# rti-team-imvia/RNb-NeuS-fork

Hardware: AMD Instinct MI355X
Metric: training rays/sec at 512 rays x 128 samples/ray (higher is better)
Workload: dtype f32; 1 GPU; DiLiGenT-MV-shaped synthetic rays, wmask_rnb.conf networks (8x256 SDF MLP + 2x256 albedo MLP), train_rnb step (render_rnb), 512 rays x (64+64) samples per GPU, 3 lights, geometric init, Adam; rays_per_gpu=512, global_rays=512, samples_per_ray=128, n_lights=3, no_albedo=False, parallelism=dp1, dp_loss=single process, deterministic=False, arithmetic=x2h, operand_bits=22, train_ops=rnb_loss_rnb + rnb_adam_step (one launch each)

## Files before the change

include/rnbneus.h:

```cpp
#ifndef RNBNEUS_H
#define RNBNEUS_H

#include <stddef.h>
#include <stdint.h>

#ifdef __cplusplus
extern "C" {
#endif

#define RNB_ABI_VERSION 5
#define RNB_MAX_LIN 16

enum {
  RNB_OK = 0,
  RNB_E_INVALID = -1,
  RNB_E_WORKSPACE = -2,
  RNB_E_HIP = -3,
  RNB_E_NULL = -4
};

typedef void* rnb_stream_t;

typedef struct rnb_model_desc {
  int32_t sdf_d_in;
  int32_t sdf_d_out;
  int32_t sdf_d_hidden;
  int32_t sdf_n_layers;
  int32_t sdf_skip_in;
  int32_t sdf_multires;
  float   sdf_scale;
  int32_t sdf_weight_norm;
  int32_t col_d_feature;
  int32_t col_d_in;
  int32_t col_d_out;
  int32_t col_d_hidden;
  int32_t col_n_layers;
  int32_t col_multires_view;
  int32_t col_squeeze_out;
  int32_t col_weight_norm;
  int32_t n_samples;
  int32_t n_importance;
  int32_t up_sample_steps;
  int32_t variant;
} rnb_model_desc;

enum {
  RNB_VARIANT_BF16 = 1,
  RNB_VARIANT_DETERMINISTIC = 2,
  RNB_VARIANT_GENERIC = 4,
  RNB_VARIANT_DW_LDS = 8,
  RNB_VARIANT_DW_STAGED = 16,
  RNB_VARIANT_X3 = 32,
  RNB_VARIANT_F32_MFMA = 64,
  RNB_VARIANT_BWD_TI_SHIFT = 8,
  RNB_VARIANT_BWD_NW_SHIFT = 10,
  RNB_VARIANT_FWD_TI_SHIFT = 12,
  RNB_VARIANT_FWD_NW_SHIFT = 14,
  RNB_VARIANT_REG_TILE = 1 << 16,
  RNB_VARIANT_LDS_TILE = 1 << 17,
  RNB_VARIANT_X2H = 1 << 18,
  RNB_VARIANT_NO_X2H = 1 << 19
};

typedef struct rnb_mlp_params {
  int32_t n_lin;
  int32_t pad_;
  const float* g[RNB_MAX_LIN];
  const float* v[RNB_MAX_LIN];
  const float* b[RNB_MAX_LIN];
} rnb_mlp_params;

typedef struct rnb_mlp_grads {
  int32_t n_lin;
  int32_t pad_;
  float* g[RNB_MAX_LIN];
  float* v[RNB_MAX_LIN];
  float* b[RNB_MAX_LIN];
} rnb_mlp_grads;

int rnb_abi_version(void);
const char* rnb_build_id(void);
const char* rnb_last_error_string(void);

int rnb_packed_floats(const rnb_model_desc* desc, int64_t* n_floats);
int rnb_weightnorm_fwd(const rnb_model_desc* desc, const rnb_mlp_params* sdf, const rnb_mlp_params* color,
                       float* packed, rnb_stream_t stream);
int rnb_weightnorm_bwd(const rnb_model_desc* desc, const rnb_mlp_params* sdf, const rnb_mlp_params* color,
                       const float* packed_grad, const rnb_mlp_grads* sdf_grads,
                       const rnb_mlp_grads* color_grads, rnb_stream_t stream);

int rnb_points_workspace_bytes(const rnb_model_desc* desc, int64_t n_points, int64_t* bytes);
int rnb_sdf_forward(const rnb_model_desc* desc, const float* packed, const float* pts, int64_t n,
                    float* sdf_out, float* feat_out, void* ws, size_t ws_bytes, rnb_stream_t stream);
int rnb_sdf_gradient(const rnb_model_desc* desc, const float* packed, const float* pts, int64_t n,
                     float* grad_out, float* sdf_out, void* ws, size_t ws_bytes, rnb_stream_t stream);
int rnb_color_forward(const rnb_model_desc* desc, const float* packed, const float* pts,
                      const float* normals, const float* feats, int64_t n, float* out, void* ws,
                      size_t ws_bytes, rnb_stream_t stream);

enum { RNB_POINTS_FEATURE = 1, RNB_POINTS_NORMAL = 2, RNB_POINTS_COLOR = 4 };
int rnb_points_grad_workspace_bytes(const rnb_model_desc* desc, int64_t n_points, int32_t flags, int64_t* bytes);
int rnb_sdf_forward_save(const rnb_model_desc* desc, const float* packed, const float* pts, int64_t n,
                         int32_t flags, float* sdf_out, float* feat_out, float* nrm_out, void* ws, size_t ws_bytes,
                         rnb_stream_t stream);
int rnb_sdf_backward(const rnb_model_desc* desc, const float* packed, int64_t n, int32_t flags, const float* sdf_bar,
                     const float* feat_bar, const float* nrm_bar, float* packed_grad, float* x_bar, void* ws,
                     size_t ws_bytes, rnb_stream_t stream);
int rnb_color_forward_save(const rnb_model_desc* desc, const float* packed, const float* pts, const float* normals,
                           const float* feats, int64_t n, float* out, void* ws, size_t ws_bytes, rnb_stream_t stream);
int rnb_color_backward(const rnb_model_desc* desc, const float* packed, int64_t n, const float* alb_bar,
                       float* packed_grad, float* feat_bar, float* nrm_bar, float* pts_bar, void* ws, size_t ws_bytes,
                       rnb_stream_t stream);

typedef struct rnb_grid_desc {
  float bound_min[3];
  float bound_max[3];
  int32_t resolution;
  int32_t x_begin, x_end;
  float out_scale;
} rnb_grid_desc;
int rnb_sdf_grid_workspace_bytes(const rnb_model_desc* desc, const rnb_grid_desc* grid, int64_t* bytes);
int rnb_sdf_grid(const rnb_model_desc* desc, const float* packed, const rnb_grid_desc* grid, float* volume,
                 void* ws, size_t ws_bytes, rnb_stream_t stream);

typedef struct rnb_sparse_grid_desc {
  int32_t brick;
  float threshold;
  float margin;
} rnb_sparse_grid_desc;
int rnb_sdf_grid_sparse_workspace_bytes(const rnb_model_desc* desc, const rnb_grid_desc* grid,
                                        const rnb_sparse_grid_desc* sparse, int64_t* bytes);
int rnb_sdf_grid_sparse_seed(const rnb_model_desc* desc, const float* packed, const rnb_grid_desc* grid,
                             const rnb_sparse_grid_desc* sparse, void* ws, size_t ws_bytes, int64_t* n_listed,
                             rnb_stream_t stream);
int rnb_sdf_grid_sparse_round(const rnb_model_desc* desc, const float* packed, const rnb_grid_desc* grid,
                              const rnb_sparse_grid_desc* sparse, float* volume, void* ws, size_t ws_bytes, int64_t first,
                              int64_t count, int64_t* n_listed, rnb_stream_t stream);
int rnb_sdf_grid_sparse_finish(const rnb_model_desc* desc, const rnb_grid_desc* grid, const rnb_sparse_grid_desc* sparse,
                               float* volume, void* ws, size_t ws_bytes, uint8_t* brick_mask, rnb_stream_t stream);

int rnb_up_sample_step(const float* rays_o, const float* rays_d, const float* z_in, const float* sdf_in,
                       int64_t B, int32_t n, int32_t n_new, float inv_s, float* new_z, int32_t* inds,
                       float* z_out, int32_t* sort_index, rnb_stream_t stream);
int rnb_gather_sdf(const float* sdf_old, const float* sdf_new, const int32_t* sort_index, int64_t B,
                   int32_t n, int32_t n_new, float* sdf_out, rnb_stream_t stream);
int rnb_sample_workspace_bytes(const rnb_model_desc* desc, int64_t B, int64_t* bytes);
int rnb_sample_rays(const rnb_model_desc* desc, const float* packed, const float* rays_o,
                    const float* rays_d, const float* near, const float* far, const float* t_rand,
                    int64_t B, float* z_vals_out, void* ws, size_t ws_bytes, rnb_stream_t stream);

enum {
  RNB_MODE_CORE = 0,
  RNB_MODE_MVPS = 1,
  RNB_FLAG_RELU_SHADING = 2,
  RNB_FLAG_NO_ALBEDO = 4,
  RNB_FLAG_LIGHT_PER_RAY = 8,
  RNB_FLAG_FORWARD_ONLY = 16,
  RNB_FLAG_INPUT_GRADS = 32
};

typedef struct rnb_render_args {
  int64_t B;
  int32_t S;
  int32_t n_lights;
  int32_t flags;
  float   cos_anneal_ratio;
  const float* rays_o;
  const float* rays_d;
  const float* z_vals;
  const float* lights_dir;
  const float* background_rgb;
  const float* variance;
// ... 106 lines not shown
```

rnb-neus-fork_amd/csrc/api.hip:

```cpp
#include <math.h>
#include <stdlib.h>

#include "rnb_internal.h"

using namespace rnb;

#define RNB_API extern "C" __attribute__((visibility("default")))

#define RNB_REQUIRE(p, name) \
  if (!(p)) RNB_FAIL(RNB_E_NULL, name " is NULL")

#if __has_include("../build/build_id.h")
#include "../build/build_id.h"
#endif
#ifndef RNB_BUILD_ID
#define RNB_BUILD_ID "unknown"
#endif

RNB_API int rnb_abi_version(void) { return RNB_ABI_VERSION; }
RNB_API const char* rnb_build_id(void) { return RNB_BUILD_ID; }
RNB_API const char* rnb_last_error_string(void) { return rnb::last_error(); }

RNB_API int rnb_packed_floats(const rnb_model_desc* desc, int64_t* n_floats) {
  RNB_REQUIRE(n_floats, "n_floats");
  Layout L;
  RNB_TRY(make_layout(desc, &L));
  *n_floats = L.total_all;
  return RNB_OK;
}

RNB_API int rnb_weightnorm_fwd(const rnb_model_desc* desc, const rnb_mlp_params* sdf, const rnb_mlp_params* color,
                               float* packed, rnb_stream_t stream) {
  RNB_REQUIRE(packed, "packed");
  Layout L;
  RNB_TRY(make_layout(desc, &L));
  RNB_TRY(weightnorm_fwd(desc, L, sdf, color, packed, (hipStream_t)stream));
  if (is_bf16(L)) RNB_TRY(bf16_pack_weights(L, packed, (hipStream_t)stream));
  if (is_x3(L)) RNB_TRY(x3_pack_weights(L, packed, (hipStream_t)stream));
  return RNB_OK;
}

RNB_API int rnb_weightnorm_bwd(const rnb_model_desc* desc, const rnb_mlp_params* sdf, const rnb_mlp_params* color,
                               const float* packed_grad, const rnb_mlp_grads* sdf_grads,
                               const rnb_mlp_grads* color_grads, rnb_stream_t stream) {
  RNB_REQUIRE(packed_grad, "packed_grad");
  Layout L;
  RNB_TRY(make_layout(desc, &L));
  return weightnorm_bwd(desc, L, sdf, color, packed_grad, sdf_grads, color_grads, (hipStream_t)stream);
}

static const int kPointsMode = PM_WITH_NORMAL | PM_WITH_COLOR;

RNB_API int rnb_points_workspace_bytes(const rnb_model_desc* desc, int64_t n_points, int64_t* bytes) {
  RNB_REQUIRE(bytes, "bytes");
  if (n_points < 0) RNB_FAIL(RNB_E_INVALID, "n_points < 0");
  Layout L;
  RNB_TRY(make_layout(desc, &L));
  Carver c(nullptr, 0);
  PointBufs pb;
  carve_points(L, c, n_points, kPointsMode, &pb);
  *bytes = (int64_t)c.off;
  return RNB_OK;
}

static int points_setup(const rnb_model_desc* desc, int64_t n, void* ws, size_t ws_bytes, Layout* L, PointBufs* pb) {
  RNB_TRY(make_layout(desc, L));
  RNB_REQUIRE(ws, "workspace");
  Carver c(ws, ws_bytes);
  carve_points(*L, c, n, kPointsMode, pb);
  if (!c.ok) RNB_FAIL(RNB_E_WORKSPACE, "workspace too small: need %zu bytes, have %zu", c.off, ws_bytes);
  pb->smax = nullptr;
  return RNB_OK;
}

static int forward_points(const Layout& L, const float* packed, const float* pts, int64_t n, PointBufs& pb,
                          bool save, bool need_feat, bool reverse_follows, float* feat_dense, hipStream_t s) {
  switch (L.route.sdf) {
    case SDF_BF16:
      RNB_TRY(bf16_forward(L, packed, pts, n, pb, save, need_feat, s, nullptr, save && need_feat && L.route.color == COLOR_BF16));
      break;
    case SDF_FUSED:
      RNB_TRY(fused_forward(L, packed, pts, n, pb, save, need_feat, s));
      break;
    case SDF_LAYERS:
      RNB_TRY(launch_pe_points(L, pts, n, pb, s));
      return sweep_forward(L, packed, pb, need_feat, reverse_follows, feat_dense, s);
  }
  if (need_feat && feat_dense) RNB_TRY(launch_copy_cols(pb.cin, L.Cinp, L.F, n, feat_dense, s));
  return RNB_OK;
}

static int reverse_points(const Layout& L, const float* packed, PointBufs& pb, bool store_ge, hipStream_t s) {
  switch (L.route.sdf) {
    case SDF_BF16: return bf16_reverse(L, packed, pb, s);
    case SDF_FUSED: return fused_reverse(L, packed, pb, s, store_ge);
    case SDF_LAYERS: break;
  }
  return sweep_reverse(L, packed, pb, s);
}

static int color_points(const Layout& L, const float* packed, PointBufs& pb, const float* pts, hipStream_t s) {
  switch (L.route.color) {
    case COLOR_BF16: return bf16_color_forward(L, packed, pb, pts, s);
    case COLOR_H2: return color_h2_forward(L, packed, pb, pts, pb.nrm, s);
    case COLOR_LAYERS: return sweep_color(L, packed, pb, pts, pb.nrm, 4, s);
    case COLOR_NONE: break;
  }
  RNB_FAIL(RNB_E_INVALID, "model has no albedo network");
}

RNB_API int rnb_sdf_forward(const rnb_model_desc* desc, const float* packed, const float* pts, int64_t n,
                            float* sdf_out, float* feat_out, void* ws, size_t ws_bytes, rnb_stream_t stream) {
  RNB_REQUIRE(packed, "packed");
  RNB_REQUIRE(pts, "pts");
  RNB_REQUIRE(sdf_out, "sdf_out");
  if (n <= 0) return n == 0 ? RNB_OK : (set_error("n < 0"), RNB_E_INVALID);
  hipStream_t s = (hipStream_t)stream;
  Layout L;
  PointBufs pb;
  RNB_TRY(points_setup(desc, n, ws, ws_bytes, &L, &pb));
  RNB_TRY(forward_points(L, packed, pts, n, pb, false, feat_out != nullptr, false, feat_out, s));
// ... 891 lines not shown
```

rnb-neus-fork_amd/csrc/backward.hip:

```cpp
#include "gemm.hip.h"
#include "rnb_internal.h"

namespace rnb {

__global__ __launch_bounds__(64) void nbar_geb_kernel(const float* __restrict__ x4, const float* __restrict__ nrm,
                                                      const float* __restrict__ nbar_in,
                                                      const float* __restrict__ cinb, int Cinp, int blk_off,
                                                      int pen_off, int multires_view, int with_color, int multires,
                                                      int Ep, int64_t M, int64_t Mp, float* __restrict__ geb,
                                                      unsigned* __restrict__ amax) {
  extern __shared__ float tile[];
  const int lane = threadIdx.x;
  const int64_t r0 = (int64_t)blockIdx.x * 64, row = r0 + lane;
  float nb[3] = {0.f, 0.f, 0.f};
  if (with_color) {
    const int Wc = Cinp - blk_off;
    tile_load64(cinb, Cinp, r0, blk_off, Wc, tile, lane);
    __builtin_amdgcn_wave_barrier();
    if (row < M) {
      const float* g = tile + lane * (Wc + 1) + (pen_off - blk_off);
#pragma unroll
      for (int d = 0; d < 3; ++d) nb[d] = nbar_in[row * 4 + d] + g[d];
      float f = 1.f;
      int c = 3;
      for (int k = 0; k < multires_view; ++k) {
#pragma unroll
        for (int d = 0; d < 3; ++d) {
          float s, co;
          sincosf(nrm[row * 4 + d] * f, &s, &co);
          nb[d] += f * (g[c + d] * co - g[c + 3 + d] * s);
        }
        c += 6;
        f *= 2.f;
      }
    }
    __builtin_amdgcn_wave_barrier();
  } else if (row < M) {
#pragma unroll
    for (int d = 0; d < 3; ++d) nb[d] = nbar_in[row * 4 + d];
  }
  float* o = tile + lane * (Ep + 1);
  o[0] = nb[0]; o[1] = nb[1]; o[2] = nb[2];
  float gm = fmaxf(fmaxf(fabsf(nb[0]), fabsf(nb[1])), fabsf(nb[2]));
  int c = 3;
  float f = 1.f;
  for (int k = 0; k < multires; ++k) {
#pragma unroll
    for (int d = 0; d < 3; ++d) {
      float s, co;
      sincosf(x4[row * 4 + d] * f, &s, &co);
      const float v0 = f * co * nb[d], v1 = -f * s * nb[d];
      o[c + d] = v0;
      o[c + 3 + d] = v1;
      gm = fmaxf(gm, fmaxf(fabsf(v0), fabsf(v1)));
    }
    c += 6;
    f *= 2.f;
  }
  for (; c < Ep; ++c) o[c] = 0.f;
  if (amax != nullptr) amax_commit(amax, gm, lane);
  __builtin_amdgcn_wave_barrier();
  tile_store64(geb, Ep, r0, 0, Ep, tile, lane);
}

__global__ __launch_bounds__(512) void sdf_head_bwd_kernel(const float* __restrict__ a, const float* __restrict__ ulast,
                                                           const float* __restrict__ ucol, int ntiles,
                                                           int Hp, int H, const float* __restrict__ sbar,
                                                           float inv_scale, int64_t M, int rows_per_blk,
                                                           float* __restrict__ dwsdf, float* __restrict__ dbsdf,
                                                           float* __restrict__ part_w, float* __restrict__ part_b) {
  __shared__ double red[64][33];
  __shared__ double redb[64];
  const int tid = threadIdx.x, cg = tid & 7, ph = tid >> 3;
  const int kl = cg * 4, k0 = blockIdx.y * 32 + kl;
  const int64_t r0 = (int64_t)blockIdx.x * rows_per_blk;
  const int64_t r1 = min(M, r0 + rows_per_blk);
  double s[4] = {0.0, 0.0, 0.0, 0.0}, sb = 0.0;
#pragma unroll 4
  for (int64_t row = r0 + ph; row < r1; row += 64) {
    const float t = sbar[row] * inv_scale;
    if (cg == 0) sb += (double)t;
    const vf4 av = *reinterpret_cast<const vf4*>(a + row * Hp + k0);
    if (ulast != nullptr) {
      const vf4 uv = *reinterpret_cast<const vf4*>(ulast + row * Hp + k0);
#pragma unroll
      for (int j = 0; j < 4; ++j) s[j] += (double)(t * av[j] + uv[j]);
    } else {
#pragma unroll
      for (int j = 0; j < 4; ++j) s[j] += (double)(t * av[j]);
    }
  }
  if (ulast == nullptr && blockIdx.x == 0) {
    for (int tile = ph; tile < ntiles; tile += 64) {
      const vf4 uv = *reinterpret_cast<const vf4*>(ucol + (size_t)tile * Hp + k0);
#pragma unroll
      for (int j = 0; j < 4; ++j) s[j] += (double)uv[j];
    }
  }
#pragma unroll
  for (int j = 0; j < 4; ++j) red[ph][kl + j] = s[j];
  if (cg == 0) redb[ph] = sb;
  __syncthreads();
  if (tid < 32) {
    double t = 0.0;
    for (int q = 0; q < 64; ++q) t += red[q][tid];
    const int col = blockIdx.y * 32 + tid;
    if (part_w != nullptr) part_w[(size_t)blockIdx.x * Hp + col] = col < H ? (float)t : 0.f;
    else if (col < H) atomicAdd(dwsdf + col, (float)t);
  } else if (tid == 32 && blockIdx.y == 0) {
    double t = 0.0;
    for (int q = 0; q < 64; ++q) t += redb[q];
    if (part_b != nullptr) part_b[blockIdx.x] = (float)t;
    else atomicAdd(dbsdf, (float)t);
  }
}

__global__ void sdf_xbar_kernel(const float* __restrict__ x4, const float* __restrict__ ebar, const float* __restrict__ ge,
                                const float* __restrict__ nbar, int Ep, int multires, float scale, int64_t M,
                                float* __restrict__ xbar) {
  const int64_t row = (int64_t)blockIdx.x * blockDim.x + threadIdx.x;
  if (row >= M) return;
  const float* eb = ebar + row * Ep;
  float acc[3] = {eb[0], eb[1], eb[2]};
  float f = 1.f;
  int c = 3;
  for (int k = 0; k < multires; ++k) {
#pragma unroll
    for (int d = 0; d < 3; ++d) {
      float sn, co;
      sincosf(x4[row * 4 + d] * f, &sn, &co);
      acc[d] += f * (eb[c + d] * co - eb[c + 3 + d] * sn);
      if (ge != nullptr) {
        const float* g = ge + row * Ep;
        acc[d] -= f * f * (g[c + d] * sn + g[c + 3 + d] * co) * nbar[row * 4 + d];
      }
    }
    c += 6;
    f *= 2.f;
  }
#pragma unroll
  for (int d = 0; d < 3; ++d) xbar[row * 3 + d] = scale * acc[d];
}

__global__ void color_input_bwd_kernel(const float* __restrict__ cinb, int Cinp, int F, int pev, int multires_view,
                                       const float* __restrict__ p4, const float* __restrict__ n4, int64_t M,
                                       float* __restrict__ pbar, float* __restrict__ nbar) {
  const int64_t row = (int64_t)blockIdx.x * blockDim.x + threadIdx.x;
  if (row >= M) return;
  for (int which = 0; which < 2; ++which) {
    float* out = which ? nbar : pbar;
    if (out == nullptr) continue;
    const float* g = cinb + row * Cinp + F + which * pev;
    const float* v = (which ? n4 : p4) + row * 4;
    float t[3] = {g[0], g[1], g[2]};
    float f = 1.f;
    int c = 3;
    for (int k = 0; k < multires_view; ++k) {
#pragma unroll
      for (int d = 0; d < 3; ++d) {
        float sn, co;
        sincosf(v[d] * f, &sn, &co);
// ... 111 lines not shown
```

rnb-neus-fork_amd/csrc/composite.hip:

```cpp
#include "rnb_internal.h"

namespace rnb {

constexpr int kMaxL = kMaxRenderLights;

__device__ inline float sigm(float x) { return 1.0f / (1.0f + expf(-x)); }

__device__ inline float inv_s_from_variance(const float* variance, bool* inside_clip) {
  const float raw = expf(variance[0] * 10.0f);
  if (inside_clip) *inside_clip = (raw >= 1e-6f) && (raw <= 1e6f);
  return clamp_nan(raw, 1e-6f, 1e6f);
}

__global__ void fine_points_kernel(const float* __restrict__ rays_o, const float* __restrict__ rays_d,
                                   const float* __restrict__ z, int64_t B, int S, float sample_dist,
                                   float* __restrict__ pts, float* __restrict__ dists, unsigned* __restrict__ smax) {
  int64_t i = (int64_t)blockIdx.x * blockDim.x + threadIdx.x;
  if (smax != nullptr && i < SMAX_SLOTS) smax[i] = 0u;
  if (i >= B * S) return;
  const int64_t b = i / S;
  const int j = (int)(i - b * S);
  const float zz = z[i];
  const float dd = j + 1 < S ? z[i + 1] - zz : sample_dist;
  const float mid = zz + dd * 0.5f;
// ... 35 lines not shown
  st.e_prev = s - ic * delta * 0.5f;
  st.pc = sigm(st.e_prev * inv_s);
  st.nc = sigm(st.e_next * inv_s);
  st.raw = (st.pc - st.nc + 1e-5f) / (st.pc + 1e-5f);
  st.alpha = clamp_nan(st.raw, 0.f, 1.f);
  return st;
}

__device__ inline void load_light(const CompArgs& a, int l, int64_t b, float (&Lv)[3]) {
  const float* p = (a.flags & RNB_FLAG_LIGHT_PER_RAY) ? a.lights + ((int64_t)l * a.B + b) * 3 : a.lights + l * 3;
  Lv[0] = p[0]; Lv[1] = p[1]; Lv[2] = p[2];
}

__global__ __launch_bounds__(64) void composite_fwd_kernel(CompArgs a) {
  const int lane = threadIdx.x;
  const int64_t b = blockIdx.x;
  const int S = a.S;
  const bool mvps = (a.flags & RNB_MODE_MVPS) != 0;
  const bool relu_sh = (a.flags & RNB_FLAG_RELU_SHADING) != 0;
  const bool no_alb = (a.flags & RNB_FLAG_NO_ALBEDO) != 0;
  const float inv_s = inv_s_from_variance(a.variance, nullptr);
  const float d0 = a.rays_d[b * 3], d1 = a.rays_d[b * 3 + 1], d2 = a.rays_d[b * 3 + 2];
  float Lv[kMaxL][3];
  if (mvps)
    for (int l = 0; l < a.L; ++l) load_light(a, l, b, Lv[l]);

  float carry = 1.0f;
  float col[kMaxL][4];
#pragma unroll
  for (int l = 0; l < kMaxL; ++l)
#pragma unroll
    for (int c = 0; c < 4; ++c) col[l][c] = 0.f;
  float wsum = 0.f, wmax = -1.f, gnum = 0.f, gden = 0.f;

  for (int j0 = 0; j0 < S; j0 += 64) {
    const int j = j0 + lane;
    const bool on = j < S;
    const int64_t p = b * S + (on ? j : S - 1);
    const float s = a.sdf[p];
    const float n0 = a.nrm[p * 4], n1 = a.nrm[p * 4 + 1], n2 = a.nrm[p * 4 + 2];
    const SampleState st = eval_sample(s, n0, n1, n2, d0, d1, d2, a.dists[p], inv_s, a.cos_anneal);
    const float x = on ? (1.0f - st.alpha + 1e-7f) : 1.0f;
    const float incl = wave_scan_mul(x, lane);
    float excl = __shfl_up(incl, 1, 64);
    if (lane == 0) excl = 1.0f;
    const float T = carry * excl;
    carry = carry * __shfl(incl, 63, 64);
    const float w = on ? st.alpha * T : 0.f;
    const float px = a.pts[p * 3], py = a.pts[p * 3 + 1], pz = a.pts[p * 3 + 2];
    const float pn = sqrtf(px * px + py * py + pz * pz);
    const float nn = sqrtf(n0 * n0 + n1 * n1 + n2 * n2);
    if (on) {
      a.weights[p] = w;
      a.cdf[p] = st.pc;
      a.gradients[p * 3] = n0; a.gradients[p * 3 + 1] = n1; a.gradients[p * 3 + 2] = n2;
      a.inside[p] = pn < 1.0f ? 1.f : 0.f;
      if (a.sdf_out) a.sdf_out[p] = s;
      if (a.albedo_out)
        for (int c = 0; c < a.C; ++c) a.albedo_out[p * a.C + c] = a.alb[p * 4 + c];
      wsum += w;
      wmax = max_nan(wmax, w);
      {
        const float relax = pn < 1.2f ? 1.f : 0.f;
        gnum += relax * ((nn - 1.0f) * (nn - 1.0f));
        gden += relax;
      }
      float al[4];
#pragma unroll
      for (int c = 0; c < 4; ++c) al[c] = no_alb ? 1.0f : a.alb[p * 4 + c];
      if (mvps) {
        for (int l = 0; l < a.L; ++l) {
          float sh = n0 * Lv[l][0] + n1 * Lv[l][1] + n2 * Lv[l][2];
          if (relu_sh) sh = relu_nan(sh);
          const float ws = w * sh;
#pragma unroll
          for (int c = 0; c < 4; ++c) col[l][c] = fmaf(al[c], ws, col[l][c]);
        }
      } else {
#pragma unroll
        for (int c = 0; c < 4; ++c) col[0][c] = fmaf(a.alb[p * 4 + c], w, col[0][c]);
      }
    }
  }
  wsum = wave_sum(wsum);
  wmax = wave_max(wmax);
  gnum = wave_sum(gnum);
  gden = wave_sum(gden);
  const int nl = mvps ? a.L : 1;
  for (int l = 0; l < nl; ++l)
    for (int c = 0; c < a.C; ++c) {
      float v = wave_sum(col[l][c]);
      if (lane == 0) {
        if (mvps) a.color_fine[((int64_t)l * a.B + b) * a.C + c] = v;
        else if (c < 3) {
          if (a.bg) v += a.bg[c] * (1.0f - wsum);
          a.color_fine[b * 3 + c] = v;
        }
      }
    }
  if (lane == 0) {
    a.weight_sum[b] = wsum;
    a.weight_max[b] = wmax;
    a.s_val[b] = 1.0f / inv_s;
    a.gerr_part[b * 2] = gnum;
    a.gerr_part[b * 2 + 1] = gden;
  }
}

__global__ __launch_bounds__(64) void composite_maps_kernel(CompMapsArgs g) {
  const CompArgs& a = g.f;
  const int lane = threadIdx.x;
  const int64_t b = blockIdx.x;
  const int S = a.S;
  const bool mvps = (a.flags & RNB_MODE_MVPS) != 0;
  const bool relu_sh = (a.flags & RNB_FLAG_RELU_SHADING) != 0;
  const bool no_alb = (a.flags & RNB_FLAG_NO_ALBEDO) != 0;
  const bool want_color = a.color_fine != nullptr;
  const float inv_s = inv_s_from_variance(a.variance, nullptr);
  const float d0 = a.rays_d[b * 3], d1 = a.rays_d[b * 3 + 1], d2 = a.rays_d[b * 3 + 2];
  float Lv[kMaxL][3];
  if (mvps && want_color)
    for (int l = 0; l < a.L; ++l) load_light(a, l, b, Lv[l]);

  float carry = 1.0f;
  float col[kMaxL][4];
#pragma unroll
  for (int l = 0; l < kMaxL; ++l)
#pragma unroll
    for (int c = 0; c < 4; ++c) col[l][c] = 0.f;
  float wsum = 0.f, wmax = -1.f;
  float nacc[3] = {0.f, 0.f, 0.f}, aacc[4] = {0.f, 0.f, 0.f, 0.f}, dacc = 0.f;

  for (int j0 = 0; j0 < S; j0 += 64) {
    const int j = j0 + lane;
    const bool on = j < S;
    const int64_t p = b * S + (on ? j : S - 1);
    const float s = a.sdf[p];
    const float n0 = a.nrm[p * 4], n1 = a.nrm[p * 4 + 1], n2 = a.nrm[p * 4 + 2];
    const SampleState st = eval_sample(s, n0, n1, n2, d0, d1, d2, a.dists[p], inv_s, a.cos_anneal);
    const float x = on ? (1.0f - st.alpha + 1e-7f) : 1.0f;
    const float incl = wave_scan_mul(x, lane);
    float excl = __shfl_up(incl, 1, 64);
    if (lane == 0) excl = 1.0f;
    const float T = carry * excl;
    carry = carry * __shfl(incl, 63, 64);
    const float w = on ? st.alpha * T : 0.f;
    const float px = a.pts[p * 3], py = a.pts[p * 3 + 1], pz = a.pts[p * 3 + 2];
    const float pn = sqrtf(px * px + py * py + pz * pz);
    if (on) {
      wsum += w;
      wmax = max_nan(wmax, w);
      if (g.normal) {
        const float wi = w * (pn < 1.0f ? 1.f : 0.f);
        nacc[0] = fmaf(wi, n0, nacc[0]); nacc[1] = fmaf(wi, n1, nacc[1]); nacc[2] = fmaf(wi, n2, nacc[2]);
      }
      if (g.albedo) {
#pragma unroll
        for (int c = 0; c < 4; ++c) aacc[c] = fmaf(a.alb[p * 4 + c], w, aacc[c]);
      }
      if (g.depth) dacc = fmaf(w, g.z[p] + a.dists[p] * 0.5f, dacc);
      if (want_color) {
        float al[4];
#pragma unroll
        for (int c = 0; c < 4; ++c) al[c] = no_alb ? 1.0f : a.alb[p * 4 + c];
        if (mvps) {
          for (int l = 0; l < a.L; ++l) {
            float sh = n0 * Lv[l][0] + n1 * Lv[l][1] + n2 * Lv[l][2];
            if (relu_sh) sh = relu_nan(sh);
            const float ws = w * sh;
#pragma unroll
            for (int c = 0; c < 4; ++c) col[l][c] = fmaf(al[c], ws, col[l][c]);
          }
        } else {
#pragma unroll
          for (int c = 0; c < 4; ++c) col[0][c] = fmaf(a.alb[p * 4 + c], w, col[0][c]);
        }
      }
    }
  }
  wsum = wave_sum(wsum);
  wmax = wave_max(wmax);
  if (want_color) {
    const int nl = mvps ? a.L : 1;
    for (int l = 0; l < nl; ++l)
      for (int c = 0; c < a.C; ++c) {
        float v = wave_sum(col[l][c]);
        if (lane == 0) {
          if (mvps) a.color_fine[((int64_t)l * a.B + b) * a.C + c] = v;
          else if (c < 3) {
            if (a.bg) v += a.bg[c] * (1.0f - wsum);
            a.color_fine[b * 3 + c] = v;
          }
        }
      }
  }
  if (g.normal) {
#pragma unroll
    for (int d = 0; d < 3; ++d) {
      const float v = wave_sum(nacc[d]);
      if (lane == 0) g.normal[b * 3 + d] = v;
    }
  }
  if (g.albedo) {
    for (int c = 0; c < a.C; ++c) {
      const float v = wave_sum(aacc[c]);
      if (lane == 0) g.albedo[b * a.C + c] = v;
    }
  }
  if (g.depth) {
    const float v = wave_sum(dacc);
    if (lane == 0) g.depth[b] = v;
  }
  if (lane == 0) {
    if (a.weight_sum) a.weight_sum[b] = wsum;
    if (a.weight_max) a.weight_max[b] = wmax;
  }
}

__global__ __launch_bounds__(256) void gerr_finalize_kernel(const float* __restrict__ part, int64_t B,
                                                            float* __restrict__ gerr, float* __restrict__ den_out,
                                                            float* __restrict__ partial) {
  __shared__ float rn[4], rd[4];
  float n = 0.f, d = 0.f;
  for (int64_t i = threadIdx.x; i < B; i += 256) { n += part[i * 2]; d += part[i * 2 + 1]; }
  n = wave_sum(n);
  d = wave_sum(d);
  if ((threadIdx.x & 63) == 0) { rn[threadIdx.x >> 6] = n; rd[threadIdx.x >> 6] = d; }
  __syncthreads();
  if (threadIdx.x == 0) {
    const float nn = rn[0] + rn[1] + rn[2] + rn[3];
    const float ds = rd[0] + rd[1] + rd[2] + rd[3];
    const float dd = ds + 1e-5f;
    gerr[0] = nn / dd;
    den_out[0] = dd;
    if (partial) { partial[0] = nn; partial[1] = ds; }
  }
}


template <bool IG>
__device__ __forceinline__ void composite_bwd_body(const CompBwdArgs& g) {
  __shared__ float sAlpha[kMaxS], sT[kMaxS], sWbar[kMaxS], sSuf[kMaxS];
  if (g.amax_to_zero != nullptr && blockIdx.x == 0) {
    static_assert(AMAX_SLOTS <= 64, "one wave zeroes the slots");
    if ((int)threadIdx.x < AMAX_SLOTS) g.amax_to_zero[threadIdx.x] = 0u;
  }
  const CompArgs& a = g.f;
  const int lane = threadIdx.x;
  const int64_t b = blockIdx.x;
  const int S = a.S;
  const bool mvps = (a.flags & RNB_MODE_MVPS) != 0;
  const bool relu_sh = (a.flags & RNB_FLAG_RELU_SHADING) != 0;
  const bool no_alb = (a.flags & RNB_FLAG_NO_ALBEDO) != 0;
  const float inv_s = inv_s_from_variance(a.variance, nullptr);
  const float c_an = a.cos_anneal;
  const float d0 = a.rays_d[b * 3], d1 = a.rays_d[b * 3 + 1], d2 = a.rays_d[b * 3 + 2];
  float Lv[kMaxL][3], Cb[kMaxL][4];
#pragma unroll
  for (int l = 0; l < kMaxL; ++l)
#pragma unroll
    for (int c = 0; c < 4; ++c) Cb[l][c] = 0.f;
  const int nl = mvps ? a.L : 1;
  if (mvps)
    for (int l = 0; l < a.L; ++l) load_light(a, l, b, Lv[l]);
  if (g.g_color) {
    for (int l = 0; l < nl; ++l)
      for (int c = 0; c < (mvps ? a.C : 3); ++c)
        Cb[l][c] = mvps ? g.g_color[((int64_t)l * a.B + b) * a.C + c] : g.g_color[b * 3 + c];
  }
  const float g_wsum = g.g_weight_sum ? g.g_weight_sum[b] : 0.f;
  const float g_wmax = g.g_weight_max ? g.g_weight_max[b] : 0.f;
  float bg_dot = 0.f;
  if (!mvps && a.bg) bg_dot = Cb[0][0] * a.bg[0] + Cb[0][1] * a.bg[1] + Cb[0][2] * a.bg[2];

  float carry = 1.0f;
  float wmax = -1.f;
  int wmax_j = 0;
  float lbar[kMaxL][3];
  float wsum_ig = 0.f;
  if constexpr (IG) {
#pragma unroll
    for (int l = 0; l < kMaxL; ++l) lbar[l][0] = lbar[l][1] = lbar[l][2] = 0.f;
  }
  for (int j0 = 0; j0 < S; j0 += 64) {
    const int j = j0 + lane;
    const bool on = j < S;
    const int64_t p = b * S + (on ? j : S - 1);
    const float n0 = a.nrm[p * 4], n1 = a.nrm[p * 4 + 1], n2 = a.nrm[p * 4 + 2];
    const SampleState st = eval_sample(a.sdf[p], n0, n1, n2, d0, d1, d2, a.dists[p], inv_s, c_an);
    const float x = on ? (1.0f - st.alpha + 1e-7f) : 1.0f;
    const float incl = wave_scan_mul(x, lane);
    float excl = __shfl_up(incl, 1, 64);
    if (lane == 0) excl = 1.0f;
    const float T = carry * excl;
    carry = carry * __shfl(incl, 63, 64);
    if (on) {
      const float w = st.alpha * T;
      float wb = g_wsum + (g.g_weights ? g.g_weights[p] : 0.f);
      float nb0 = 0.f, nb1 = 0.f, nb2 = 0.f;
      float ab[4] = {0.f, 0.f, 0.f, 0.f};
      float al[4];
#pragma unroll
      for (int c = 0; c < 4; ++c) al[c] = (mvps && no_alb) ? 1.0f : a.alb[p * 4 + c];
      if (mvps) {
        for (int l = 0; l < a.L; ++l) {
          const float sh_raw = n0 * Lv[l][0] + n1 * Lv[l][1] + n2 * Lv[l][2];
          const float sh = relu_sh ? fmaxf(sh_raw, 0.f) : sh_raw;
          float ca = 0.f;
#pragma unroll
          for (int c = 0; c < 4; ++c) {
            ca = fmaf(Cb[l][c], al[c], ca);
            ab[c] = fmaf(Cb[l][c], w * sh, ab[c]);
          }
          wb = fmaf(ca, sh, wb);
          float shb = ca * w;
          if (relu_sh && !(sh_raw > 0.f)) shb = 0.f;
          nb0 = fmaf(shb, Lv[l][0], nb0); nb1 = fmaf(shb, Lv[l][1], nb1); nb2 = fmaf(shb, Lv[l][2], nb2);
          if constexpr (IG) if (g.ig_light) { lbar[l][0] = fmaf(shb, n0, lbar[l][0]); lbar[l][1] = fmaf(shb, n1, lbar[l][1]); lbar[l][2] = fmaf(shb, n2, lbar[l][2]); }
        }
        if (no_alb) { ab[0] = ab[1] = ab[2] = ab[3] = 0.f; }
      } else {
#pragma unroll
        for (int c = 0; c < 3; ++c) { wb = fmaf(Cb[0][c], al[c], wb); ab[c] = Cb[0][c] * w; }
        wb -= bg_dot;
      }
      sAlpha[j] = st.alpha;
      sT[j] = T;
      sWbar[j] = wb;
      g.nbar[p * 4] = nb0; g.nbar[p * 4 + 1] = nb1; g.nbar[p * 4 + 2] = nb2; g.nbar[p * 4 + 3] = 0.f;
#pragma unroll
      for (int c = 0; c < 4; ++c) g.albbar[p * 4 + c] = ab[c];
      if (w > wmax) { wmax = w; wmax_j = j; }
      if constexpr (IG) wsum_ig += w;
    }
  }
  if constexpr (IG) {
    if (g.ig_light) {
      for (int l = 0; l < a.L; ++l)
#pragma unroll
        for (int d = 0; d < 3; ++d) {
          const float v = wave_sum(lbar[l][d]);
          if (lane == 0) g.ig_light[((int64_t)l * a.B + b) * 3 + d] = v;
        }
    }
    if (g.ig_bg) {
      const float ws = wave_sum(wsum_ig);
      if (lane == 0)
        for (int c = 0; c < 3; ++c) g.ig_bg[b * 3 + c] = Cb[0][c] * (1.0f - ws);
    }
  }
  if (g.g_weight_max) {
    const float m = wave_max(wmax);
    int cand = (wmax == m) ? wmax_j : 0x7fffffff;
#pragma unroll
    for (int o = 32; o > 0; o >>= 1) cand = min(cand, __shfl_xor(cand, o, 64));
    __syncthreads();
    if (lane == 0 && cand < S) sWbar[cand] += g_wmax;
  }
  __syncthreads();
  if (lane == 0) {
    double run = 0.0;
    for (int j = S - 1; j >= 0; --j) {
      sSuf[j] = (float)run;
      run += (double)sWbar[j] * (double)(sAlpha[j] * sT[j]);
    }
  }
  __syncthreads();
  const float gerr_coef = g.g_gerr ? g.g_gerr[0] / (g.gerr_den_global ? g.gerr_den_global[0] : g.gerr_den[0]) : 0.f;
  float invs_bar = 0.f;
  float cosd0 = 0.f, cosd1 = 0.f, cosd2 = 0.f;
  for (int j0 = 0; j0 < S; j0 += 64) {
    const int j = j0 + lane;
    if (j >= S) continue;
    const int64_t p = b * S + j;
    const float n0 = a.nrm[p * 4], n1 = a.nrm[p * 4 + 1], n2 = a.nrm[p * 4 + 2];
    const float delta = a.dists[p];
    const SampleState st = eval_sample(a.sdf[p], n0, n1, n2, d0, d1, d2, delta, inv_s, c_an);
    float alphabar = sWbar[j] * sT[j] - sSuf[j] / (1.0f - st.alpha + 1e-7f);
    const float rawbar = (st.raw >= 0.f && st.raw <= 1.f) ? alphabar : 0.f;
    const float den = st.pc + 1e-5f;
    float pcbar = rawbar * (1.0f / den - (st.pc - st.nc + 1e-5f) / (den * den));
    const float ncbar = -rawbar / den;
    if (g.g_cdf) pcbar += g.g_cdf[p];
    float epb = pcbar * st.pc * (1.0f - st.pc);
    float enb = ncbar * st.nc * (1.0f - st.nc);
    invs_bar += epb * st.e_prev + enb * st.e_next;
    epb *= inv_s;
    enb *= inv_s;
    g.sbar[p] = epb + enb;
    const float icbar = (enb - epb) * delta * 0.5f;
    const float tcbar = icbar * (((-st.tc * 0.5f + 0.5f) > 0.f ? 0.5f * (1.0f - c_an) : 0.f) +
                                 ((-st.tc) > 0.f ? c_an : 0.f));
    if constexpr (IG) if (g.ig_cos_d) { cosd0 = fmaf(tcbar, n0, cosd0); cosd1 = fmaf(tcbar, n1, cosd1); cosd2 = fmaf(tcbar, n2, cosd2); }
    if constexpr (IG) if (g.ig_dists) {
      const float ic = -(relu_nan(-st.tc * 0.5f + 0.5f) * (1.0f - c_an) + relu_nan(-st.tc) * c_an);
      g.ig_dists[p] = (enb - epb) * ic * 0.5f;
    }
    float nb0 = g.nbar[p * 4] + tcbar * d0, nb1 = g.nbar[p * 4 + 1] + tcbar * d1, nb2 = g.nbar[p * 4 + 2] + tcbar * d2;
    if (g.g_gerr) {
      const float px = a.pts[p * 3], py = a.pts[p * 3 + 1], pz = a.pts[p * 3 + 2];
      if (sqrtf(px * px + py * py + pz * pz) < 1.2f) {
        const float nn = sqrtf(n0 * n0 + n1 * n1 + n2 * n2);
        if (nn > 0.f) {
          const float k = gerr_coef * 2.0f * (nn - 1.0f) / nn;
          nb0 = fmaf(k, n0, nb0); nb1 = fmaf(k, n1, nb1); nb2 = fmaf(k, n2, nb2);
        }
      }
    }
    if (g.g_gradients) {
      nb0 += g.g_gradients[p * 3]; nb1 += g.g_gradients[p * 3 + 1]; nb2 += g.g_gradients[p * 3 + 2];
    }
    g.nbar[p * 4] = nb0; g.nbar[p * 4 + 1] = nb1; g.nbar[p * 4 + 2] = nb2;
  }
  invs_bar = wave_sum(invs_bar);
  if (lane == 0) {
    if (g.g_s_val) invs_bar -= g.g_s_val[b] / (inv_s * inv_s);
    g.invs_part[b] = invs_bar;
  }
  if constexpr (IG) if (g.ig_cos_d) {
    cosd0 = wave_sum(cosd0);
    cosd1 = wave_sum(cosd1);
    cosd2 = wave_sum(cosd2);
    if (lane == 0) { g.ig_cos_d[b * 3] = cosd0; g.ig_cos_d[b * 3 + 1] = cosd1; g.ig_cos_d[b * 3 + 2] = cosd2; }
  }
}

__global__ __launch_bounds__(64) void composite_bwd_kernel(CompBwdArgs g) { composite_bwd_body<false>(g); }
__global__ __launch_bounds__(64) void composite_bwd_ig_kernel(CompBwdArgs g) { composite_bwd_body<true>(g); }

__global__ __launch_bounds__(64) void ray_input_adjoint_kernel(RayAdjArgs r) {
  const int lane = threadIdx.x;
  const int64_t b = blockIdx.x;
  const int S = r.S;
  const float d0 = r.rays_d[b * 3], d1 = r.rays_d[b * 3 + 1], d2 = r.rays_d[b * 3 + 2];
  float ob[3] = {0.f, 0.f, 0.f}, db[3] = {0.f, 0.f, 0.f};
  float carry_D = 0.f;
  for (int j0 = 0; j0 < S; j0 += 64) {
    const int j = j0 + lane;
    const bool on = j < S;
    const int64_t p = b * S + (on ? j : S - 1);
    float nt[3], pb[3];
#pragma unroll
    for (int d = 0; d < 3; ++d) nt[d] = r.nbar[p * 4 + d];
    if (r.cinb != nullptr) {
      const float* gn = r.cinb + p * r.Cinp + r.F + r.pev;
      const float* gp = r.cinb + p * r.Cinp + r.F;
#pragma unroll
// ... 151 lines not shown
```

rnb-neus-fork_amd/csrc/dw.hip.h:

```cpp
#pragma once
#include "gemm.hip.h"

namespace rnb {

struct DwPair {
  const float* X;
  int ldx;
  const float* Y;
  int ldy;
  int adj = 0;
  const unsigned* amax = nullptr;
  const unsigned* smax = nullptr;
};

template <bool GUARD, int KT>
__device__ inline void dw_main_loop(const DwPair& p, int m_begin, int m_end, int N, int K, int n_blk, int k_blk,
                                    int wm, int wn, unsigned mask, bool do_bias, double& bsum,
                                    float* __restrict__ Xs, float* __restrict__ Ys, v16f (&acc)[2][KT / 64]) {
  const int tid = threadIdx.x, lane = tid & 63;
  vf4 rx[4], ry[KT / 32];
  load_kmajor<128, GUARD>(p.X, p.ldx, m_begin, n_blk, m_end, N, tid, rx);
  load_kmajor<KT, GUARD>(p.Y, p.ldy, m_begin, k_blk, m_end, K, tid, ry);
  for (int m0 = m_begin; m0 < m_end; m0 += BK) {
    store_kmajor<128>(Xs, tid, rx);
// ... 180 lines not shown
    for (int c = 0; c < nch; c += 3) {
      RNB_DW_LOAD(2, c + 2)
      __builtin_amdgcn_sched_barrier(0);
      RNB_DW_MMA(0)
      __builtin_amdgcn_sched_barrier(0);
      RNB_DW_LOAD(0, c + 3)
      __builtin_amdgcn_sched_barrier(0);
      if (c + 1 < nch) RNB_DW_MMA(1)
      __builtin_amdgcn_sched_barrier(0);
      RNB_DW_LOAD(1, c + 4)
      __builtin_amdgcn_sched_barrier(0);
      if (c + 2 < nch) RNB_DW_MMA(2)
      __builtin_amdgcn_sched_barrier(0);
    }
#undef RNB_DW_LOAD
#undef RNB_DW_MMA
  }
  float* __restrict__ dW = J.dW;
  const int lddw = J.lddw;
  float* __restrict__ pdst = J.part ? J.part + (size_t)split * N * lddw : nullptr;
#pragma unroll
  for (int tj = 0; tj < TN; ++tj) {
    const int col = k_w + tj * 32 + i;
#pragma unroll
    for (int ti = 0; ti < 2; ++ti) {
#pragma unroll
      for (int r = 0; r < 16; ++r) {
        const int row = n_w + 2 * ((r & 3) + 8 * (r >> 2) + 4 * h) + ti;
        if (pdst) pdst[(size_t)row * lddw + col] = acc[ti][tj][r];
        else atomicAdd(dW + (size_t)row * lddw + col, acc[ti][tj][r]);
      }
    }
  }
  if (bias_wave) {
    bs0 += __shfl_xor(bs0, 32, 64);
    bs1 += __shfl_xor(bs1, 32, 64);
    if (h == 0) {
      if (J.partb) {
        J.partb[(size_t)split * N + n_w + 2 * i] = (float)bs0;
        J.partb[(size_t)split * N + n_w + 2 * i + 1] = (float)bs1;
      } else {
        atomicAdd(J.db + n_w + 2 * i, (float)bs0);
        atomicAdd(J.db + n_w + 2 * i + 1, (float)bs1);
      }
    }
  }
}

template <int DUMMY>
__global__ __launch_bounds__(256) void dw_reduce_kernel(const DwGroup g) {
  const DwJob& J = g.job[blockIdx.y];
  const size_t n = (size_t)J.N * J.K;
  const bool dense = J.K == J.lddw;
  if (J.splits > 64) {
    __shared__ double red[16][17];
    const size_t ntot = n + ((J.db != nullptr && J.partb != nullptr) ? (size_t)J.N : 0);
    const int e = threadIdx.x & 15, ph = threadIdx.x >> 4;
    for (size_t base = (size_t)blockIdx.x * 16; base < ntot; base += (size_t)gridDim.x * 16) {
      const size_t idx = base + e;
      double s[4] = {0.0, 0.0, 0.0, 0.0};
      if (idx < ntot) {
        const float* src = idx < n ? J.part + idx : J.partb + (idx - n);
        const size_t stride = idx < n ? n : (size_t)J.N;
        int sp = ph;
        for (; sp + 48 < J.splits; sp += 64) {
#pragma unroll
          for (int u = 0; u < 4; ++u) s[u] += (double)src[(size_t)(sp + 16 * u) * stride];
        }
        for (int u = 0; sp < J.splits; sp += 16, ++u) s[u] += (double)src[(size_t)sp * stride];
      }
      red[ph][e] = (s[0] + s[1]) + (s[2] + s[3]);
      __syncthreads();
      if (threadIdx.x < 16 && base + threadIdx.x < ntot) {
        const size_t i2 = base + threadIdx.x;
        double t = 0.0;
        for (int q = 0; q < 16; ++q) t += red[q][threadIdx.x];
        if (i2 < n) J.dW[dense ? i2 : (i2 / (size_t)J.K) * (size_t)J.lddw + i2 % (size_t)J.K] = (float)t;
        else J.db[i2 - n] = (float)t;
      }
      __syncthreads();
    }
    return;
  }
  for (size_t idx = (size_t)blockIdx.x * 256 + threadIdx.x; idx < n; idx += (size_t)gridDim.x * 256) {
    double s[4] = {0.0, 0.0, 0.0, 0.0};
    int sp = 0;
    for (; sp + 4 <= J.splits; sp += 4) {
#pragma unroll
      for (int u = 0; u < 4; ++u) s[u] += (double)J.part[(size_t)(sp + u) * n + idx];
    }
    for (int u = 0; sp < J.splits; ++sp, ++u) s[u] += (double)J.part[(size_t)sp * n + idx];
    const size_t dst = dense ? idx : (idx / (size_t)J.K) * (size_t)J.lddw + idx % (size_t)J.K;
    J.dW[dst] = (float)((s[0] + s[1]) + (s[2] + s[3]));
  }
  if (J.db != nullptr && J.partb != nullptr) {
    for (int r = blockIdx.x * 256 + threadIdx.x; r < J.N; r += gridDim.x * 256) {
      double s = 0.0;
      for (int sp = 0; sp < J.splits; ++sp) s += (double)J.partb[(size_t)sp * J.N + r];
      J.db[r] = (float)s;
    }
  }
}

constexpr int kStChunk = 32;
constexpr int kStOpBytes = kStChunk * 256 * 4;
constexpr int kStBufs = 2;

__device__ inline void dw_staged_issue(const DwPair& p, int m_begin, int nchunks, int chunk, char* buf, int wave, int lane) {
  const int c = chunk < nchunks ? chunk : nchunks - 1;
#pragma unroll
  for (int q = 0; q < kStChunk / 16; ++q) {
    const int u = (q * 16 + wave) * 64 + lane;
    const int row = m_begin + c * kStChunk + (u >> 6);
    const float* xs = p.X + (size_t)row * p.ldx + (u & 63) * 4;
    const float* ys = p.Y + (size_t)row * p.ldy + (u & 63) * 4;
    __builtin_amdgcn_global_load_lds((const __attribute__((address_space(1))) void*)xs,
                                     (__attribute__((address_space(3))) void*)(buf + (q * 16 + wave) * 1024), 16, 0, 0);
    __builtin_amdgcn_global_load_lds((const __attribute__((address_space(1))) void*)ys,
                                     (__attribute__((address_space(3))) void*)(buf + kStOpBytes + (q * 16 + wave) * 1024), 16, 0, 0);
  }
}

template <int DUMMY>
__global__ __launch_bounds__(1024, 1) void gemm_dw_staged_kernel(const DwGroup g) {
  __shared__ __attribute__((aligned(16))) char lds[kStBufs * 2 * kStOpBytes];
  const int tid = threadIdx.x, lane = tid & 63;
  const int wave = wave_id();
  const int wm = wave >> 2, wn = wave & 3;
  int ji = 0, begin = 0;
  for (int q = 0; q + 1 < g.njobs; ++q)
    if ((int)blockIdx.x >= g.job[q].block_end) { ji = q + 1; begin = g.job[q].block_end; }
  const DwJob& J = g.job[ji];
  const int split = (int)blockIdx.x - begin;
  if (split >= J.splits) return;
  const int m_begin = split * J.rows_per_split;
  const int m_end = min(g.M, m_begin + J.rows_per_split);
  if (m_begin >= m_end) return;
  const int nchunks = (m_end - m_begin) / kStChunk;
  const int i = lane & 31, h = lane >> 5;
  v16f acc[2][2];
  zero_acc<2>(acc);
  double bs0 = 0.0, bs1 = 0.0;
  const bool bias_wave = J.db != nullptr && wn == 0;
  for (int pi = 0; pi < J.npairs; ++pi) {
    const DwPair p = pi == 0 ? J.p1 : J.p2;
    const bool do_bias = bias_wave && pi == J.bias_pair;
    __builtin_amdgcn_s_barrier();
    dw_staged_issue(p, m_begin, nchunks, 0, lds, wave, lane);
    for (int c = 0; c < nchunks; ++c) {
      asm volatile("s_waitcnt vmcnt(0)" ::: "memory");
      __builtin_amdgcn_s_barrier();
      dw_staged_issue(p, m_begin, nchunks, c + 1, lds + ((c + 1) & 1) * 2 * kStOpBytes, wave, lane);
      const char* bx = lds + (c & 1) * 2 * kStOpBytes;
      const char* by = bx + kStOpBytes;
      float t0 = 0.f, t1 = 0.f;
      const char* ax = bx + h * 1024 + (wm * 64 + 2 * i) * 4;
      const char* ay = by + h * 1024 + (wn * 64 + i) * 4;
      vf2 a0 = *reinterpret_cast<const vf2*>(ax);
      float b00 = *reinterpret_cast<const float*>(ay), b01 = *reinterpret_cast<const float*>(ay + 128);
#pragma unroll
      for (int q = 0; q < kStChunk / 2; q += 2) {
        const vf2 a1 = *reinterpret_cast<const vf2*>(ax + (q + 1) * 2048);
        const float b10 = *reinterpret_cast<const float*>(ay + (q + 1) * 2048);
        const float b11 = *reinterpret_cast<const float*>(ay + (q + 1) * 2048 + 128);
        __builtin_amdgcn_sched_barrier(0);
        acc[0][0] = __builtin_amdgcn_mfma_f32_32x32x2f32(a0.x, b00, acc[0][0], 0, 0, 0);
        acc[1][0] = __builtin_amdgcn_mfma_f32_32x32x2f32(a0.y, b00, acc[1][0], 0, 0, 0);
        acc[0][1] = __builtin_amdgcn_mfma_f32_32x32x2f32(a0.x, b01, acc[0][1], 0, 0, 0);
        acc[1][1] = __builtin_amdgcn_mfma_f32_32x32x2f32(a0.y, b01, acc[1][1], 0, 0, 0);
        if (do_bias) { t0 += a0.x; t1 += a0.y; }
        __builtin_amdgcn_sched_barrier(0);
        if (q + 2 < kStChunk / 2) {
          a0 = *reinterpret_cast<const vf2*>(ax + (q + 2) * 2048);
          b00 = *reinterpret_cast<const float*>(ay + (q + 2) * 2048);
          b01 = *reinterpret_cast<const float*>(ay + (q + 2) * 2048 + 128);
        }
        __builtin_amdgcn_sched_barrier(0);
        acc[0][0] = __builtin_amdgcn_mfma_f32_32x32x2f32(a1.x, b10, acc[0][0], 0, 0, 0);
        acc[1][0] = __builtin_amdgcn_mfma_f32_32x32x2f32(a1.y, b10, acc[1][0], 0, 0, 0);
        acc[0][1] = __builtin_amdgcn_mfma_f32_32x32x2f32(a1.x, b11, acc[0][1], 0, 0, 0);
        acc[1][1] = __builtin_amdgcn_mfma_f32_32x32x2f32(a1.y, b11, acc[1][1], 0, 0, 0);
// ... 288 lines not shown
```

rnb-neus-fork_amd/csrc/fused.hip:

```cpp
#include <type_traits>

#include "fused_common.hip.h"

#ifndef RNB_X3_SCALAR_EPI
#define RNB_X3_SCALAR_EPI 0
#endif
#ifndef RNB_H2_SCALAR_EPI
#define RNB_H2_SCALAR_EPI 1
#endif
#ifndef RNB_H2_GUARD_AB
#define RNB_H2_GUARD_AB 0
#endif

namespace rnb {


template <int TI, bool SAVE, int NW = 4, bool X3 = false, bool H2 = false>
__global__ __launch_bounds__(64 * NW, NW == 8 ? 1 : 2) void fused_forward_kernel(FusedFwdArgs g) {
  static_assert(!H2 || X3, "x2h is a form of the split-operand path");
  constexpr float SA = H2 ? kH2ActScale : 1.f;
  constexpr int WP = H2 ? 2 : 3;
  constexpr int FT = 32 * TI;
  constexpr int NT = 64 * NW;
  constexpr int TJ = 8 / NW;
// ... 144 lines not shown
              D = vf2{0.f, 0.f};
              if constexpr (H2) am = fmaxf(am, fmaxf(fabsf(a.x), fabsf(a.y)));
            }
          }
          Y[row * FP + col] = a.x * SA;
          Y[(row + 1) * FP + col] = a.y * SA;
          if constexpr (H2 && RNB_H2_GUARD_AB != 1) h2_track2(amb, a.x, a.y);
          if (SAVE) {
            bstore(ra, voff, rowc * FH * 4, a.x);
            bstore(ra, voff, (rowc + 1) * FH * 4, a.y);
            bstore(rD, voff, rowc * FH * 4, D.x);
            bstore(rD, voff, (rowc + 1) * FH * 4, D.y);
          }
        }
      }
    };
#pragma unroll
    for (int tj = 0; tj < TJ; ++tj) {
      if (n0 + tj * 32 + 32 <= n_real) column_tile(std::true_type{}, tj);
      else column_tile(std::false_type{}, tj);
    }
    if constexpr (H2 && RNB_H2_GUARD_AB != 1) {
      am = fmaxf(am, __builtin_bit_cast(float, amb));
      h2_raise_flag(am, &ovf[l & 1], lane);
    }
    lds_barrier();
    if constexpr (H2) {
      sa = SA;
      isa = 1.f / SA;
      am_prev = am;
    }
    if constexpr (NBUF == 2) { float* t = X; X = Y; Y = t; }
  }
  if constexpr (H2 && RNB_H2_GUARD_AB == 0) {
    if (h2_flag_up(&ovf[(g.net.nh - 1) & 1])) rescale_input(am_prev, g.net.nh - 1);
  }

  {
    const float* ws = g.packed + g.net.wsdf_off;
    float w[4];
#pragma unroll
    for (int u = 0; u < 4; ++u) w[u] = ws[lane + 64 * u];
    const float bs = g.packed[g.net.bsdf_off];
    for (int rr = 0; rr < FT / NW; ++rr) {
      const int row = wave * (FT / NW) + rr;
      float s = 0.f;
#pragma unroll
      for (int u = 0; u < 4; ++u) s = fmaf(X[row * FP + lane + 64 * u], w[u], s);
#pragma unroll
      for (int o = 32; o > 0; o >>= 1) s += __shfl_xor(s, o, 64);
      if (lane == 0) {
        const float v = (H2 ? __builtin_fmaf(s, isa, bs) : s + bs) / g.net.scale;
        sweep_store_sdf(g.grid, g.sdf, row0, row, g.M, v);
      }
    }
  }
  if (g.with_feat) {
    [[maybe_unused]] const float inv = H2 ? isa * h2_iws_at(iwsv, g.net.nh) : 1.f;
    if constexpr (X3) mm.run(X, g.w3 + WP * g.net.wf_off, FH, n0, lane, acc, nullptr, 0, 0);
    else layer_mma_nt<TI, NoHook, TJ>(X, g.packed + g.net.wf_off, FH, n0, lane, acc);
    const float* bias = g.packed + g.net.bf_off;
    const BufRsrc rc = tile_rsrc(g.cin + (size_t)row0 * g.net.Cinp, FT * g.net.Cinp * 4);
    const unsigned rowb = (unsigned)g.net.Cinp * 4u;
#pragma unroll
    for (int tj = 0; tj < TJ; ++tj) {
      const int col = n0 + tj * 32 + cl;
      if (col < g.net.F) {
        const float bc = bias[col];
        const unsigned voff = (unsigned)(4 * h) * rowb + (unsigned)col * 4u;
#pragma unroll
        for (int ti = 0; ti < TI; ++ti) {
#pragma unroll
          for (int r = 0; r < 16; ++r) {
            const int rowc = ti * 32 + (r & 3) + 8 * (r >> 2);
            bstore(rc, voff, rowc * rowb, H2 ? __builtin_fmaf(acc[ti][tj][r], inv, bc) : acc[ti][tj][r] + bc);
          }
        }
      }
    }
  }
}

constexpr int kMaxX3 = 4 * RNB_MAX_LIN + 2;
struct X3Entry { long long off; int N, K, unit_begin, tperm, id, tr; };
struct X3Table { int n, total_units; X3Entry e[kMaxX3]; };
__global__ __launch_bounds__(256) void x3_pack_kernel(const float* __restrict__ src, X3Table t, x3raw* __restrict__ dst,
                                                      H2Tab* __restrict__ tab) {
  __shared__ float wmx[4];
  const int u = blockIdx.x * 256 + threadIdx.x;
  const bool live = u < t.total_units;
  int ei = 0;
  while (ei + 1 < t.n && u >= t.e[ei + 1].unit_begin) ++ei;
  const X3Entry en = t.e[ei];
  float m = 0.f;
  if (live) {
    const int lu = u - en.unit_begin;
    const int frag = lu >> 6, lane = lu & 63;
    const int nks = en.K >> 4;
    const int nt = frag / nks, ks = frag - nt * nks;
    const int c = lane & 31, h = lane >> 5;
    const float* sp = src + en.off + (size_t)(nt * 32 + c) * en.K + ks * 16 + h * (en.tperm ? 4 : 8);
    const vf4 x0 = *reinterpret_cast<const vf4*>(sp), x1 = *reinterpret_cast<const vf4*>(sp + (en.tperm ? 8 : 4));
    vu4x hi, mid, lo;
    x3_split8(x0, x1, hi, mid, lo);
    x3raw* dp = dst + 3 * en.off + ((size_t)frag * 3 * 64 + lane) * 8;
    *reinterpret_cast<vu4x*>(dp) = hi;
    *reinterpret_cast<vu4x*>(dp + 512) = mid;
    *reinterpret_cast<vu4x*>(dp + 1024) = lo;
    m = fmaxf(fmaxf(fmaxf(fabsf(x0.x), fabsf(x0.y)), fmaxf(fabsf(x0.z), fabsf(x0.w))),
              fmaxf(fmaxf(fabsf(x1.x), fabsf(x1.y)), fmaxf(fabsf(x1.z), fabsf(x1.w))));
  }
  if (tab == nullptr) return;
  const bool rec = live && en.id >= 0 && !en.tr;
  const int blk0 = blockIdx.x * 256;
  const bool whole = en.unit_begin <= blk0 && blk0 + 256 <= en.unit_begin + en.N * en.K / 8;
#pragma unroll
  for (int o = 32; o > 0; o >>= 1) m = fmaxf(m, __shfl_xor(m, o, 64));
  if (!whole) {
    if (rec && (threadIdx.x & 63) == 0) amax_tile_commit(tab->wmax + en.id, m);
    return;
  }
  if ((threadIdx.x & 63) == 0) wmx[threadIdx.x >> 6] = m;
  __syncthreads();
  if (rec && threadIdx.x == 0) amax_tile_commit(tab->wmax + en.id, fmaxf(fmaxf(wmx[0], wmx[1]), fmaxf(wmx[2], wmx[3])));
}
__device__ inline float x2h_weight_scale(unsigned mbits, float& inv) {
  float s = kH2WScale;
  inv = 1.f / kH2WScale;
  const int ef = (int)(mbits >> 23);
  if (ef >= 127 + 6 && ef < 255) x2h_dyn_scale(mbits, s, inv);
  return s;
}
__global__ void x2h_pack_kernel(const float* __restrict__ src, X3Table t, x3raw* __restrict__ dst, H2Tab* __restrict__ tab) {
  const int u = blockIdx.x * blockDim.x + threadIdx.x;
  if (u >= t.total_units) return;
  int ei = 0;
  while (ei + 1 < t.n && u >= t.e[ei + 1].unit_begin) ++ei;
  const X3Entry en = t.e[ei];
  const int lu = u - en.unit_begin;
  const int frag = lu >> 6, lane = lu & 63;
  const int nks = en.K >> 4;
  const int nt = frag / nks, ks = frag - nt * nks;
  const int c = lane & 31, h = lane >> 5;
  float inv;
  const float sw = x2h_weight_scale(tab->wmax[en.id], inv);
  if (lu == 0 && !en.tr) { tab->ws[en.id] = sw; tab->iws[en.id] = inv; }
  const float* sp = src + en.off + (size_t)(nt * 32 + c) * en.K + ks * 16 + h * (en.tperm ? 4 : 8);
  vu4x hi, lo;
  x2h_split8(*reinterpret_cast<const vf4*>(sp) * sw, *reinterpret_cast<const vf4*>(sp + (en.tperm ? 8 : 4)) * sw, hi, lo);
  x3raw* dp = dst + 2 * en.off + ((size_t)frag * 2 * 64 + lane) * 8;
  *reinterpret_cast<vu4x*>(dp) = hi;
  *reinterpret_cast<vu4x*>(dp + 512) = lo;
}
int x3_pack_weights(const Layout& L, float* packed, hipStream_t s) {
  x3raw* dst = reinterpret_cast<x3raw*>(packed + L.total);
  X3Table t;
  t.n = 0;
  t.total_units = 0;
  auto add = [&](long long off, int N, int K, int tperm, int id, int tr) {
    if (off < 0 || N <= 0 || K <= 0) return;
    X3Entry& e = t.e[t.n++];
    e.off = off; e.N = N; e.K = K; e.unit_begin = t.total_units; e.tperm = tperm; e.id = id; e.tr = tr;
    t.total_units += N * K / 8;
  };
  for (int l = 0; l < L.nh; ++l) {
    add(L.hid[l].w_off, L.hid[l].Np, L.hid[l].Kp, 1, l, 0);
    add(L.hid[l].wT_off, L.hid[l].Kp, L.hid[l].Np, 1, l, 1);
  }
  if (L.F > 0) {
    add(L.feat.w_off, L.feat.Np, L.feat.Kp, 1, L.nh, 0);
    add(L.feat.wT_off, L.feat.Kp, L.feat.Np, 1, L.nh, 1);
  }
  for (int l = 0; l < L.nc; ++l) {
    add(L.col[l].w_off, L.col[l].Np, L.col[l].Kp, 0, L.nh + 1 + l, 0);
    add(L.col[l].wT_off, L.col[l].Kp, L.col[l].Np, 0, L.nh + 1 + l, 1);
  }
  H2Tab* tab = is_x2h(L) ? h2_tab(L, packed) : nullptr;
  hipLaunchKernelGGL(x3_pack_kernel, dim3((unsigned)((t.total_units + 255) / 256)), dim3(256), 0, s, packed, t, dst, tab);
  RNB_CHECK_LAUNCH();
  if (is_x2h(L)) {
    for (int q = 0; q < t.n; ++q) t.e[q].tperm = 1;
    hipLaunchKernelGGL(x2h_pack_kernel, dim3((unsigned)((t.total_units + 255) / 256)), dim3(256), 0, s, packed, t,
                       x2h_mirror(L, packed), tab);
    RNB_CHECK_LAUNCH();
  }
  return RNB_OK;
}

bool fused_supported(const Layout& L) {
  if (L.Hp != FH || L.H != FH) return false;
  if (L.Ep > 64 || L.pe > FEP) return false;
  if (L.nh < 1) return false;
  for (int l = 0; l < L.nh; ++l)
    if (L.hid[l].Np != FH || (L.hid[l].Kp != FH && l != 0)) return false;
  if (L.F > FH || (L.F > 0 && L.Fp != FH)) return false;
  return true;
}

int fused_forward(const Layout& L, const float* packed, const float* pts, int64_t M, PointBufs& pb, bool save,
                  bool need_feat, hipStream_t s, const GridGen* grid) {
  const int64_t fam_rows = family_rows_of(grid, pb.Mp);
  if (!save && use_reg_tile(L, fam_rows)) return sweep_mv_forward(L, packed, pts, M, pb, save, need_feat, s, grid);
  const bool h2 = is_x2h(L);
  FusedFwdArgs g;
  memset(&g, 0, sizeof(g));
  g.net = sdf_net_args(L);
  if (grid) g.grid = *grid;
  g.pts = pts;
  g.M = M;
  g.packed = packed;
  g.w3 = h2 ? x2h_mirror(L, packed) : reinterpret_cast<const x3raw*>(packed + L.total);
  for (int l = 0; l < L.nh; ++l) {
    g.a[l] = pb.a[l];
    g.D[l] = pb.D[l];
  }
  g.with_feat = need_feat ? 1 : 0;
  g.cin = pb.cin;
  g.sdf = pb.sdf;
  g.x4 = pb.x;
  g.e = pb.e;
  g.h2tab = h2 ? h2_tab(L, packed) : nullptr;
  g.smax = (save && h2) ? pb.smax : nullptr;
  ProfScope prof(sdf_sweep_flops(L, M, 0, true, need_feat), s, save ? "F_sweep(save)" : "F_sweep(forward_only)");
  const int force_ti = L.knob(RNB_VARIANT_FWD_TI_SHIFT);
  const bool small = force_ti ? (force_ti == 1) : (fam_rows / 64 < 512);
  const int force_nw = L.knob(RNB_VARIANT_FWD_NW_SHIFT);
  const bool wide = force_nw ? (force_nw == 2) : (fam_rows / 32 <= 256);
  pick_c<1, 0>(save, [&](auto save_c) {
    pick_c<2, 1, 0>(h2 ? 2 : is_x3(L) ? 1 : 0, [&](auto ar_c) {
      auto launch = [&](auto ti_c, auto nw_c) {
        constexpr int TI = decltype(ti_c)::value, NW = decltype(nw_c)::value, AR = decltype(ar_c)::value;
        hipLaunchKernelGGL((fused_forward_kernel<TI, decltype(save_c)::value != 0, NW, AR >= 1, AR == 2>),
                           dim3((unsigned)(pb.Mp / (32 * TI))), dim3(64 * NW), 0, s, g);
      };
      if (!small) launch(std::integral_constant<int, 2>{}, std::integral_constant<int, 4>{});
      else pick_c<8, 4>(wide ? 8 : 4, [&](auto nw_c) { launch(std::integral_constant<int, 1>{}, nw_c); });
    });
  });
  RNB_CHECK_LAUNCH();
  return RNB_OK;
}

}
```

rnb-neus-fork_amd/csrc/fused_bwd.hip:

```cpp
#include "fused_common.hip.h"

namespace rnb {


struct FusedBwdArgs {
  const float* packed;
  const x3raw* w3;
  SdfNetArgs net;
  float* D[RNB_MAX_LIN];
  float* gz[RNB_MAX_LIN];
  float* u[RNB_MAX_LIN + 1];
  long long M;
  float* ucol;
  float* zR[RNB_MAX_LIN];
  float* zb[RNB_MAX_LIN];
  const float* x4;
  float* nrm;
  const float* geb;
  const float* sbar;
  const float* fbar;
  int ld_fbar;
  unsigned* amax;
  const H2Tab* h2tab;
  unsigned* smax;
// ... 432 lines not shown
  for (int l = g.net.nh - 1; l >= 0; --l) {
    const int lane_e = opaque_lane(lane);
    const int h = lane_e >> 5;
    const int n_real = g.net.n_real[l];
    const bool head = (l == g.net.nh - 1);
    const int par = l & 1;
    const BufRsrc rzb = tile_rsrc(g.zb[l] + (size_t)row0 * FH, BT * FH * 4);
    if (head) {
      for_each_acc<TI, TJ>(n0, lane_e, [&](int tj, int ti, int r, int col, int rowc, int row) {
        acc[ti][tj][r] = fmaf(g.sbar[row0 + row] * g.net.inv_scale, g.packed[g.net.wsdf_off + col], acc[ti][tj][r] * unscale);
      });
      unscale = 1.f;
    }
    for_each_acc_split<TI, TJ>(
        n0, lane_e, n_real,
        [&](int tj, int ti, int r, int col, int rowc, int row) {
          const float zb = fmaf(acc[ti][tj][r] * unscale, aD.v[ti][tj][r], aZ.v[ti][tj][r]);
          bstore(rzb, (unsigned)(4 * h * FH + col) * 4u, rowc * FH * 4, zb);
          acc[ti][tj][r] = zb;
        },
        [&](int tj, int ti, int r, int col, int rowc, int row) {
          const float zb = col < n_real ? fmaf(acc[ti][tj][r] * unscale, aD.v[ti][tj][r], aZ.v[ti][tj][r]) : 0.f;
          bstore(rzb, (unsigned)(4 * h * FH + col) * 4u, rowc * FH * 4, zb);
          acc[ti][tj][r] = zb;
        });
    {
      const float mr = wave_max(acc_absmax<TI, TJ>(acc, lane_e, rows_ok));
      if (lane_e == 0) wm[par][wave] = mr;
    }
    lds_barrier();
    float s, inv;
    const float tmax = tile_scale<NW>(wm[par], s, inv);
    if (tid == 0 && g.amax != nullptr) amax_tile_commit(g.amax + AMAX_ZB + l, tmax);
    if (l == 0) break;
    for_each_acc<TI, TJ>(n0, lane_e, [&](int tj, int ti, int r, int col, int rowc, int row) {
      X[row * FP + col] = acc[ti][tj][r] * s;
    });
    lds_barrier();
    if constexpr (LATE) {
      mm.request(g.w3 + 2 * g.net.wT_off[l], FH, n0, lane);
      mm.run(X, g.w3 + 2 * g.net.wT_off[l], FH, n0, lane, acc, nullptr, 0, 0);
      prefetch_tile<TI, TJ>(g.D[l - 1], row0, n0, opaque_lane(lane), aD);
      prefetch_tile<TI, TJ>(g.zR[l - 1], row0, n0, opaque_lane(lane), aZ);
    } else {
      mm.run(X, g.w3 + 2 * g.net.wT_off[l], FH, n0, lane, acc, l > 1 ? g.w3 + 2 * g.net.wT_off[l - 1] : nullptr, FH, n0, [&]() {
        prefetch_tile<TI, TJ>(g.D[l - 1], row0, n0, lane, aD);
        prefetch_tile<TI, TJ>(g.zR[l - 1], row0, n0, lane, aZ);
      });
    }
    unscale = inv * h2_iws_at(iwsv, l);
  }
}

static void fill_args(const Layout& L, const float* packed, PointBufs& pb, FusedBwdArgs& g) {
  memset(&g, 0, sizeof(g));
  g.net = sdf_net_args(L);
  g.packed = packed;
  g.w3 = reinterpret_cast<const x3raw*>(packed + L.total);
  for (int l = 0; l < L.nh; ++l) {
    g.D[l] = pb.D[l];
    g.gz[l] = pb.gz[l];
    g.zR[l] = pb.zR[l];
    g.zb[l] = pb.zb[l];
  }
  for (int l = 1; l <= L.nh; ++l) g.u[l] = pb.u[l];
  g.M = pb.M;
  g.x4 = pb.x;
  g.nrm = pb.nrm;
  g.geb = pb.geb;
  g.sbar = pb.sbar;
  g.amax = is_x2h(L) ? pb.amax : nullptr;
  g.h2tab = is_x2h(L) ? h2_tab(L, packed) : nullptr;
}

template <class F>
static void pick_tile(const Layout& L, const PointBufs& pb, F&& f) {
  const int kt = L.knob(RNB_VARIANT_BWD_TI_SHIFT), kw = L.knob(RNB_VARIANT_BWD_NW_SHIFT);
  const int ti = kt == 1 || kt == 2 ? kt : (is_x3(L) ? 2 : 1), nw = kw == 1 ? 4 : kw == 2 ? 8 : (is_x3(L) ? 4 : 8);
  pick_c<2, 1>(ti, [&](auto ti_c) {
    pick_c<8, 4>(nw, [&](auto nw_c) { f(ti_c, nw_c, dim3((unsigned)(pb.Mp / (32 * ti_c))), dim3(64 * nw_c)); });
  });
}

int fused_reverse(const Layout& L, const float* packed, PointBufs& pb, hipStream_t s, bool store_ge) {
  FusedBwdArgs g;
  fill_args(L, packed, pb, g);
  g.ge_out = store_ge ? pb.ge : nullptr;
  if (is_x2h(L)) {
    g.w3 = x2h_mirror(L, packed);
    g.smax = pb.smax;
  }
  ProfScope prof(sdf_sweep_flops(L, pb.M, 0, false, false), s, "R_sweep");
  pick_tile(L, pb, [&](auto ti_c, auto nw_c, dim3 grid, dim3 block) {
    pick_c<2, 1, 0>(is_x2h(L) ? 2 : is_x3(L) ? 1 : 0, [&](auto ar_c) {
      constexpr int AR = decltype(ar_c)::value;
      hipLaunchKernelGGL((fused_reverse_kernel<decltype(ti_c)::value, decltype(nw_c)::value, AR >= 1, AR == 2>), grid, block, 0, s, g);
    });
  });
  RNB_CHECK_LAUNCH();
  return RNB_OK;
}

int fused_ra(const Layout& L, const float* packed, PointBufs& pb, hipStream_t s, int* u_tiles) {
  FusedBwdArgs g;
  fill_args(L, packed, pb, g);
  ProfScope prof(sdf_sweep_flops(L, pb.M, 0, false, false), s, "RA_sweep");
  pick_tile(L, pb, [&](auto ti_c, auto nw_c, dim3 grid, dim3 block) {
    if (u_tiles != nullptr) {
      g.ucol = pb.u[L.nh];
      *u_tiles = (int)grid.x;
    }
    pick_c<1, 0>(is_x3(L), [&](auto x3_c) {
      hipLaunchKernelGGL((fused_ra_kernel<decltype(ti_c)::value, decltype(nw_c)::value, decltype(x3_c)::value != 0>), grid, block, 0, s, g);
    });
  });
  RNB_CHECK_LAUNCH();
  return RNB_OK;
}

int fused_fb(const Layout& L, const float* packed, PointBufs& pb, bool with_color, hipStream_t s) {
  FusedBwdArgs g;
  fill_args(L, packed, pb, g);
  g.fbar = with_color ? pb.cinb : nullptr;
  g.ld_fbar = L.Cinp;
  ProfScope prof(sdf_sweep_flops(L, pb.M, 1, false, with_color), s, "FB_sweep");
  pick_tile(L, pb, [&](auto ti_c, auto nw_c, dim3 grid, dim3 block) {
    constexpr int TI = decltype(ti_c)::value, NW = decltype(nw_c)::value;
    if constexpr (TI == 2) {
      if (is_x2h(L)) {
        g.w3 = x2h_mirror(L, packed);
        hipLaunchKernelGGL((fused_fb_h2_kernel<NW>), grid, block, 0, s, g);
        return;
      }
    }
    pick_c<1, 0>(is_x3(L), [&](auto x3_c) {
      hipLaunchKernelGGL((fused_fb_kernel<TI, NW, decltype(x3_c)::value != 0>), grid, block, 0, s, g);
    });
  });
  RNB_CHECK_LAUNCH();
  return RNB_OK;
}

}
```

rnb-neus-fork_amd/csrc/layers.hip:

```cpp
#include "gemm.hip.h"
#include "rnb_internal.h"

namespace rnb {


__global__ void pe_points_kernel(const float* __restrict__ pts, int64_t M, int64_t Mp, float scale, int multires,
                                 int Ep, float* __restrict__ x4, float* __restrict__ e) {
  int64_t row = (int64_t)blockIdx.x * blockDim.x + threadIdx.x;
  if (row >= Mp) return;
  float x[3] = {0.f, 0.f, 0.f};
  if (row < M) {
    x[0] = pts[row * 3 + 0] * scale;
    x[1] = pts[row * 3 + 1] * scale;
    x[2] = pts[row * 3 + 2] * scale;
  }
  x4[row * 4 + 0] = x[0]; x4[row * 4 + 1] = x[1]; x4[row * 4 + 2] = x[2]; x4[row * 4 + 3] = 0.f;
  float* er = e + row * Ep;
  er[0] = x[0]; er[1] = x[1]; er[2] = x[2];
  int c = 3;
  float f = 1.f;
  for (int k = 0; k < multires; ++k) {
#pragma unroll
    for (int d = 0; d < 3; ++d) {
      float s, co;
// ... 361 lines not shown
#pragma unroll
      for (int c = 0; c < 4; ++c) v[c] = fmaf(sb, w[c], v[c]);
    }
    vf4 zb;
#pragma unroll
    for (int c = 0; c < 4; ++c) zb[c] = col + c < n_real ? fmaf(v[c], Dv[c], zr[c]) : 0.f;
    st4(zb_prev + o, zb);
  }
};
struct EpiReluMask {
  const float* ac_prev;
  float* out;
  int ld;
  int n_real;
  __device__ void apply4(int row, int col, vf4 v) const {
    const size_t o = (size_t)row * ld + col;
    const vf4 a = ld4(ac_prev + o);
    vf4 r;
#pragma unroll
    for (int c = 0; c < 4; ++c) r[c] = (col + c < n_real && a[c] > 0.f) ? v[c] : 0.f;
    st4(out + o, r);
  }
};
struct EpiStore {
  float* out;
  int ld;
  __device__ void apply4(int row, int col, vf4 v) const { st4(out + (size_t)row * ld + col, v); }
};

struct EpiSkipPE {
  float* ebar;
  int Ep, k_split, pe;
  __device__ void apply4(int row, int col, vf4 v) const {
#pragma unroll
    for (int c = 0; c < 4; ++c) {
      const int cc = col + c;
      if (cc >= k_split && cc < k_split + pe) ebar[(size_t)row * Ep + (cc - k_split)] = v[c];
    }
  }
};


template <bool B_KMAJOR, class Epi>
static int launch_rows(const float* A, int lda, const float* W, int ldw, int64_t Mp, int N, int K, const Epi& epi,
                       double flops, hipStream_t s, bool x3 = false, const x3raw* W3 = nullptr, unsigned* amax = nullptr,
                       int64_t m_real = 0, const char* tag = "layer_gemm") {
  ProfScope prof(flops, s, tag);
  if constexpr (!B_KMAJOR) {
    if (x3 && W3 != nullptr && N % 32 == 0 && N <= 512 && K % 32 == 0 && Mp % 128 == 0) {
      if (N <= 256) hipLaunchKernelGGL((gemm_rows_x3m_kernel<1, Epi>), dim3((unsigned)(Mp / 128)), dim3(512), 0, s, A, lda, W3, N, K, epi, amax, (long long)m_real);
      else hipLaunchKernelGGL((gemm_rows_x3m_kernel<2, Epi>), dim3((unsigned)(Mp / 128)), dim3(512), 0, s, A, lda, W3, N, K, epi, amax, (long long)m_real);
      RNB_CHECK_LAUNCH();
      return RNB_OK;
    }
    if (amax != nullptr) RNB_FAIL(RNB_E_INVALID, "layer GEMM %d x %d: the x2h maxima were requested from a kernel that does not record them", N, K);
    if (x3 && N >= 256 && K % XK == 0) {
      dim3 grid((unsigned)(Mp / BM), (unsigned)((N + 255) / 256));
      if (N % 256 == 0) hipLaunchKernelGGL((gemm_rows_x3_kernel<256, false, Epi>), grid, dim3(256), 0, s, A, lda, W, ldw, N, K, epi);
      else hipLaunchKernelGGL((gemm_rows_x3_kernel<256, true, Epi>), grid, dim3(256), 0, s, A, lda, W, ldw, N, K, epi);
      RNB_CHECK_LAUNCH();
      return RNB_OK;
    }
  }
  if (N >= 256) {
    dim3 grid((unsigned)(Mp / BM), (unsigned)((N + 255) / 256));
    if (N % 256 == 0)
      hipLaunchKernelGGL((gemm_rows_kernel<B_KMAJOR, 256, false, Epi>), grid, dim3(256), 0, s, A, lda, W, ldw, N, K, epi);
    else
      hipLaunchKernelGGL((gemm_rows_kernel<B_KMAJOR, 256, true, Epi>), grid, dim3(256), 0, s, A, lda, W, ldw, N, K, epi);
  } else {
    dim3 grid((unsigned)(Mp / BM), (unsigned)((N + 127) / 128));
    if (N % 128 == 0)
      hipLaunchKernelGGL((gemm_rows_kernel<B_KMAJOR, 128, false, Epi>), grid, dim3(256), 0, s, A, lda, W, ldw, N, K, epi);
    else
      hipLaunchKernelGGL((gemm_rows_kernel<B_KMAJOR, 128, true, Epi>), grid, dim3(256), 0, s, A, lda, W, ldw, N, K, epi);
  }
  RNB_CHECK_LAUNCH();
  return RNB_OK;
}

static inline const x3raw* x3_mirror(const Layout& L, const float* packed, int64_t off) {
  if (!is_x3(L) || off < 0) return nullptr;
  return reinterpret_cast<const x3raw*>(packed + L.total) + 3 * off;
}

int launch_pe_points(const Layout& L, const float* pts, int64_t M, PointBufs& pb, hipStream_t s) {
  hipLaunchKernelGGL(pe_points_kernel, dim3(blocks_for(pb.Mp, 256)), dim3(256), 0, s, pts, M, pb.Mp, L.sdf_scale,
                     L.multires, L.Ep, pb.x, pb.e);
  RNB_CHECK_LAUNCH();
  return RNB_OK;
}

int sweep_forward(const Layout& L, const float* packed, PointBufs& pb, bool need_feat, bool need_gz_last,
                  float* feat_dense, hipStream_t s) {
  for (int l = 0; l < L.nh; ++l) {
    const Lin& ln = L.hid[l];
    const float* in = l == 0 ? pb.e : pb.a[l - 1];
    const int lda = l == 0 ? L.Ep : L.Hp;
    EpiF epi{packed + ln.b_off, pb.a[l], pb.D[l], L.Hp, ln.N, (l + 1 == L.skip) ? pb.e : nullptr, L.Ep, L.pe};
    RNB_TRY((launch_rows<false, EpiF>(in, lda, packed + ln.w_off, ln.Kp, pb.Mp, ln.Np, ln.Kp, epi, mm_flops(pb.M, ln), s)));
  }
  hipLaunchKernelGGL(sdf_head_kernel, dim3(blocks_for(pb.Mp * 32, 256)), dim3(256), 0, s, pb.a[L.nh - 1],
                     pb.D[L.nh - 1], L.Hp, L.H, packed + L.wsdf_off, packed + L.bsdf_off, 1.f / L.sdf_scale, pb.Mp, pb.sdf,
                     need_gz_last ? pb.gz[L.nh - 1] : nullptr);
  RNB_CHECK_LAUNCH();
  if (need_feat) {
    EpiBias epi{packed + L.feat.b_off, pb.cin, L.Cinp, L.F};
    RNB_TRY((launch_rows<false, EpiBias>(pb.a[L.nh - 1], L.Hp, packed + L.feat.w_off, L.feat.Kp, pb.Mp, L.feat.Np,
                                         L.feat.Kp, epi, mm_flops(pb.M, L.feat), s)));
    if (feat_dense) {
      RNB_TRY(launch_copy_cols(pb.cin, L.Cinp, L.F, pb.M, feat_dense, s));
    }
  }
  return RNB_OK;
}

int sweep_reverse(const Layout& L, const float* packed, PointBufs& pb, hipStream_t s) {
  for (int l = L.nh - 1; l >= 1; --l) {
    const Lin& ln = L.hid[l];
    const bool is_skip = (l == L.skip);
    EpiR epi{pb.D[l - 1], pb.gz[l - 1], L.Hp, is_skip ? ln.K - L.pe : ln.K, is_skip ? pb.ge : nullptr, L.Ep, L.pe};
    RNB_TRY((launch_rows<true, EpiR>(pb.gz[l], L.Hp, packed + ln.w_off, ln.Kp, pb.Mp, ln.Kp, ln.Np, epi, mm_flops(pb.M, ln), s)));
  }
  {
    const Lin& ln = L.hid[0];
    EpiR0 epi{pb.ge, L.Ep, L.pe, L.skip >= 1 ? 1 : 0};
    RNB_TRY((launch_rows<true, EpiR0>(pb.gz[0], L.Hp, packed + ln.w_off, ln.Kp, pb.Mp, ln.Kp, ln.Np, epi, mm_flops(pb.M, ln), s)));
  }
  hipLaunchKernelGGL(normal_kernel, dim3(blocks_for(pb.Mp, 256)), dim3(256), 0, s, pb.x, pb.ge, L.Ep, L.multires,
                     pb.Mp, pb.nrm);
  RNB_CHECK_LAUNCH();
  return RNB_OK;
}

int sweep_color(const Layout& L, const float* packed, PointBufs& pb, const float* pts, const float* nrm, int nrm_ld,
                hipStream_t s) {
  hipLaunchKernelGGL(color_input_kernel, dim3(blocks_for(pb.Mp, 64)), dim3(64),
                     (size_t)64 * (L.Cinp - L.F + 1) * sizeof(float), s, pts, nrm, nrm_ld, pb.M, pb.Mp,
                     L.F, L.multires_view, L.Cinp, pb.cin);
  RNB_CHECK_LAUNCH();
  for (int l = 0; l < L.nc; ++l) {
    const Lin& ln = L.col[l];
    const float* in = l == 0 ? pb.cin : pb.ac[l - 1];
    const int lda = l == 0 ? L.Cinp : L.Hcp;
    EpiRelu epi{packed + ln.b_off, pb.ac[l], L.Hcp, ln.N};
    RNB_TRY((launch_rows<false, EpiRelu>(in, lda, packed + ln.w_off, ln.Kp, pb.Mp, ln.Np, ln.Kp, epi, mm_flops(pb.M, ln), s, is_x3(L),
                                         x3_mirror(L, packed, ln.w_off), nullptr, 0, "layer_gemm(forward)")));
    if (L.route.h2 && pb.smax != nullptr) {
      if (l == 0) RNB_TRY(launch_absmax_rows(pb.cin, pb.Mp * L.Cinp, pb.smax + SMAX_CIN, s));
      RNB_TRY(launch_absmax_rows(pb.ac[l], pb.Mp * L.Hcp, pb.smax + SMAX_AC + l, s));
    }
  }
  hipLaunchKernelGGL(color_out_kernel, dim3(blocks_for(pb.Mp * 16, 256)), dim3(256), 0, s, pb.ac[L.nc - 1], L.Hcp,
                     L.Hc, packed + L.colo.w_off, L.colo.Kp, packed + L.colo.b_off, L.Co, L.squeeze, pb.Mp, pb.alb);
  RNB_CHECK_LAUNCH();
  return RNB_OK;
}

int layers_color_backward(const Layout& L, const float* packed, PointBufs& pb, float* packed_grad, hipStream_t s) {
  const int64_t M = pb.M, Mp = pb.Mp;
  const bool det = (L.variant & RNB_VARIANT_DETERMINISTIC) != 0;
  const int chunks = L.Hcp / 32;
  int64_t slabs = det ? 1 : (256 + chunks - 1) / chunks;
  int rows_per_blk = (int)((M + slabs - 1) / slabs);
  rows_per_blk = (rows_per_blk + 63) / 64 * 64;
  hipLaunchKernelGGL(color_out_bwd_kernel, dim3(blocks_for(M, rows_per_blk), chunks), dim3(512), 0, s, pb.albbar, pb.alb,
// ... 66 lines not shown
```

rnb-neus-fork_amd/csrc/rnb_internal.h:

```cpp
#pragma once
#include <hip/hip_runtime.h>
#include <stdint.h>
#include <stdio.h>
#include <string.h>

#include <type_traits>

#include "../../include/rnbneus.h"

namespace rnb {

constexpr int kPad = 32;
constexpr int kRowPad = 128;
inline int pad32(int x) { return (x + kPad - 1) / kPad * kPad; }
inline int64_t pad_rows(int64_t m) { return (m + kRowPad - 1) / kRowPad * kRowPad; }
inline unsigned blocks_for(int64_t n, int per) { return (unsigned)((n + per - 1) / per); }

void set_error(const char* fmt, ...);
#define RNB_FAIL(code, ...)        \
  do {                             \
    ::rnb::set_error(__VA_ARGS__); \
    return (code);                 \
  } while (0)
#define RNB_CHECK_HIP(expr)                                                          \
// ... 276 lines not shown

int launch_pe_points(const Layout& L, const float* pts, int64_t M, PointBufs& pb, hipStream_t s);
int sweep_forward(const Layout& L, const float* packed, PointBufs& pb, bool need_feat, bool need_gz_last,
                  float* feat_dense, hipStream_t s);
int sweep_reverse(const Layout& L, const float* packed, PointBufs& pb, hipStream_t s);
int sweep_color(const Layout& L, const float* packed, PointBufs& pb, const float* pts, const float* nrm, int nrm_ld,
                hipStream_t s);
int layers_color_backward(const Layout& L, const float* packed, PointBufs& pb, float* packed_grad, hipStream_t s);
int layers_ra(const Layout& L, const float* packed, PointBufs& pb, hipStream_t s);
int layers_fb(const Layout& L, const float* packed, PointBufs& pb, bool with_feat, hipStream_t s);
int launch_sdf_ebar(const Layout& L, const float* packed, PointBufs& pb, float** ebar, hipStream_t s);

int launch_copy_cols(const float* src, int ld, int ncols, int64_t M, float* out, hipStream_t s);
int launch_fill_cols(const float* src, int ncols, int64_t M, int64_t Mp, int ld, float* dst, hipStream_t s);
int launch_grid_points(const GridGen& g, int64_t first, int64_t n, float* pts, hipStream_t s);
int launch_scale_copy(const float* src, float scale, int64_t n, float* dst, hipStream_t s);
int launch_grid_scatter(const GridGen& g, const float* src, int64_t first, int64_t n, float* dst, hipStream_t s);

struct SparseGeom {
  int res, bs, nb, nl;
  float thr;
  float seed_dist;
};
int launch_sparse_classify(const SparseGeom& sg, const float* lattice, uint32_t* state, int32_t* list, int64_t* n_listed,
                           hipStream_t s);
int launch_sparse_grow(const SparseGeom& sg, const float* volume, int64_t first, int64_t count, uint32_t* state, int32_t* list,
                       int64_t* n_listed, hipStream_t s);
int launch_sparse_fill(const SparseGeom& sg, const float* lattice, const uint32_t* state, float* volume, hipStream_t s);
int launch_absmax_rows(const float* x, int64_t n, unsigned* slot, hipStream_t s);
int launch_range_report(const Layout& L, const float* packed, const PointBufs& pb, bool with_color, bool with_backward, float* out,
                        hipStream_t s);

struct BwdParts {
  bool albedo;
  bool sdf;
  bool feat;
  bool normal;
  bool color_inputs;
  static BwdParts render(bool with_color, bool keep_color_inputs) { return {with_color, true, with_color, true, keep_color_inputs}; }
  static BwdParts sdf_points(bool feat, bool normal) { return {false, true, feat, normal, false}; }
  static BwdParts color_points(bool inputs) { return {true, false, false, false, inputs}; }
};
int sweep_backward(const Layout& L, const float* packed, PointBufs& pb, bool with_color, float* packed_grad, hipStream_t s);
int sweep_backward_parts(const Layout& L, const float* packed, PointBufs& pb, const BwdParts& parts, float* packed_grad,
                         hipStream_t s);
int launch_sdf_xbar(const Layout& L, const float* packed, PointBufs& pb, bool with_normal, float* xbar, hipStream_t s);
int launch_color_input_bwd(const Layout& L, const PointBufs& pb, float* pts_bar, float* nrm_bar, hipStream_t s);
int64_t dw_workspace_floats(const Layout& L, int64_t M, bool with_color);
bool dw_one_wg_runs(const Layout& L, int64_t M);
int dw_zero_partials(const Layout& L, const PointBufs& pb, const BwdParts& parts, hipStream_t s);
int dw_backward(const Layout& L, const PointBufs& pb, const BwdParts& parts, int sdfh_slabs, float* packed_grad, hipStream_t s);
int fused_reverse(const Layout& L, const float* packed, PointBufs& pb, hipStream_t s, bool store_ge = false);
int fused_ra(const Layout& L, const float* packed, PointBufs& pb, hipStream_t s, int* u_tiles = nullptr);
int fused_fb(const Layout& L, const float* packed, PointBufs& pb, bool with_color, hipStream_t s);

bool fused_supported(const Layout& L);
int fused_forward(const Layout& L, const float* packed, const float* pts, int64_t M, PointBufs& pb, bool save,
                  bool need_feat, hipStream_t s, const GridGen* grid = nullptr);
bool sweep_mv_supported(const Layout& L);
int sweep_mv_forward(const Layout& L, const float* packed, const float* pts, int64_t M, PointBufs& pb, bool save,
                     bool need_feat, hipStream_t s, const GridGen* grid = nullptr);
constexpr bool kRegTileDefault = false;
inline bool use_reg_tile(const Layout& L, int64_t Mp) {
  if (!sweep_mv_supported(L) || (L.variant & RNB_VARIANT_LDS_TILE)) return false;
  if (L.variant & RNB_VARIANT_REG_TILE) return true;
  return kRegTileDefault && Mp >= 128 * 200;
}

inline bool is_x3(const Layout& L) { return (L.variant & RNB_VARIANT_X3) != 0; }
inline bool is_x2h(const Layout& L) { return is_x3(L) && (L.variant & RNB_VARIANT_X2H) != 0; }
inline unsigned short* x2h_mirror(const Layout& L, float* packed) {
  return reinterpret_cast<unsigned short*>(packed + L.total + L.total / 2 * 3);
}
inline const unsigned short* x2h_mirror(const Layout& L, const float* packed) {
  return reinterpret_cast<const unsigned short*>(packed + L.total + L.total / 2 * 3);
}
inline const H2Tab* h2_tab(const Layout& L, const float* packed) {
  return L.h2tab_off >= 0 ? reinterpret_cast<const H2Tab*>(packed + L.h2tab_off) : nullptr;
}
inline H2Tab* h2_tab(const Layout& L, float* packed) {
  return L.h2tab_off >= 0 ? reinterpret_cast<H2Tab*>(packed + L.h2tab_off) : nullptr;
}
int x3_pack_weights(const Layout& L, float* packed, hipStream_t s);

bool color_h2_supported(const Layout& L);
int color_h2_forward(const Layout& L, const float* packed, PointBufs& pb, const float* pts, const float* nrm, hipStream_t s);
int color_h2_backward(const Layout& L, const float* packed, PointBufs& pb, hipStream_t s, bool sdf = true, bool keep_pe = false);
int64_t color_h2_part_floats(const Layout& L, int64_t M);
constexpr int kSdfHeadSlabs = 64;

inline bool is_bf16(const Layout& L) { return (L.variant & RNB_VARIANT_BF16) != 0; }
int bf16_pack_weights(const Layout& L, float* packed, hipStream_t s);
int bf16_forward(const Layout& L, const float* packed, const float* pts, int64_t M, PointBufs& pb, bool save, bool need_feat,
                 hipStream_t s, const GridGen* grid = nullptr, bool feat_k8 = false);
int bf16_reverse(const Layout& L, const float* packed, PointBufs& pb, hipStream_t s);
bool bf16_color_supported(const Layout& L);
int bf16_color_forward(const Layout& L, const float* packed, PointBufs& pb, const float* pts, hipStream_t s);
int bf16_color_backward(const Layout& L, const float* packed, PointBufs& pb, float* packed_grad, hipStream_t s);
int bf16_backward(const Layout& L, const float* packed, PointBufs& pb, bool with_color, float* packed_grad, hipStream_t s);
int64_t bf16_dw_floats(const Layout& L, int64_t M, bool with_color);

int launch_up_sample_step(const float* rays_o, const float* rays_d, const float* z_in, const float* sdf_old,
                          const float* sdf_new, const int32_t* gather_index, int n_old_for_gather,
                          int64_t B, int n, int n_new, float inv_s, float* new_z, int32_t* inds,
                          float* z_out, int32_t* sort_index, float* new_pts, float* sdf_sorted_out,
                          hipStream_t s);

struct CompArgs {
  int64_t B;
  int S, L, C;
  int flags;
  float cos_anneal;
  const float* rays_d;
  const float* pts;
  const float* dists;
  const float* sdf;
  const float* nrm;
  const float* alb;
  const float* lights;
  const float* bg;
  const float* variance;
  float* color_fine;
  float* weights;
  float* cdf;
  float* gradients;
  float* inside;
  float* weight_sum;
  float* weight_max;
  float* s_val;
  float* gerr_part;
  float* gerr;
  float* gerr_den;
  float* gerr_partial;
  float* sdf_out;
  float* albedo_out;
};

struct CompBwdArgs {
  CompArgs f;
  const float* weights;
  const float* g_color;
  const float* g_weights;
  const float* g_cdf;
  const float* g_gradients;
  const float* g_weight_sum;
  const float* g_weight_max;
  const float* g_s_val;
  const float* g_gerr;
  const float* gerr_den;
  const float* gerr_den_global;
  float* sbar;
  float* nbar;
  float* albbar;
  float* invs_part;
  float* dvar;
  unsigned* amax_to_zero;
  float* ig_cos_d;
  float* ig_light;
  float* ig_bg;
  float* ig_dists;
};

struct CompMapsArgs {
  CompArgs f;
  const float* z;
  float* normal;
// ... 67 lines not shown
```

rnb-neus-fork_amd/csrc/sampling.hip:

```cpp
#include "rnb_internal.h"

namespace rnb {


__device__ inline float sigmoidf_ref(float x) { return 1.0f / (1.0f + expf(-x)); }

__device__ inline bool scan_safe(double v, float f) {
  return (float)(v * (1.0 - 2e-13)) == f && (float)(v * (1.0 + 2e-13)) == f;
}

__device__ inline bool lt_total(float a, float b) { return a < b || (a == a && b != b); }

__global__ void z_init_kernel(const float* __restrict__ rays_o, const float* __restrict__ rays_d,
                              const float* __restrict__ near, const float* __restrict__ far,
                              const float* __restrict__ t_rand, int64_t B, int n, float* __restrict__ z,
                              float* __restrict__ pts) {
  int64_t i = (int64_t)blockIdx.x * blockDim.x + threadIdx.x;
  if (i >= B * n) return;
  const int64_t b = i / n;
  const int j = (int)(i - b * n);
  const float lin = linspace_at(0.f, 1.f, n, j);
  float zz = near[b] + (far[b] - near[b]) * lin;
  if (t_rand != nullptr) {
    const float tr = t_rand[b] - 0.5f;
// ... 91 lines not shown
    if (__any(!safe)) {
      if (lane == 0) {
        double r = 1.0;
        for (int j = 0; j < m; ++j) {
          const float al = w[j];
          const float T = (float)r;
          r *= (double)(1.0f - al + 1e-7f);
          cs[j] = al * T + 1e-5f;
        }
      }
    }
  }
  __syncthreads();
  double part = 0.0;
  for (int j = lane; j < m; j += 64) part += (double)cs[j];
#pragma unroll
  for (int o = 32; o > 0; o >>= 1) part += __shfl_xor(part, o, 64);
  const float wsum = (float)part;
  for (int j = lane; j < m; j += 64) w[j] = cs[j] / wsum;
  __syncthreads();
  {
    double loc = 0.0;
    for (int j = j0; j < j1; ++j) loc += (double)w[j];
    double inc = loc;
#pragma unroll
    for (int o = 1; o < 64; o <<= 1) {
      const double t = __shfl_up(inc, o, 64);
      if (lane >= o) inc += t;
    }
    double run = __shfl_up(inc, 1, 64);
    if (lane == 0) { run = 0.0; cdf[0] = 0.f; }
    bool safe = true;
    for (int j = j0; j < j1; ++j) {
      const float wj = w[j];
      safe = safe && (wj >= 7.450580596923828e-09f) && (wj < 4.0f);
      run += (double)wj;
      cdf[j + 1] = (float)run;
    }
    if (__any(!safe)) {
      if (lane == 0) {
        double r = 0.0;
        for (int j = 0; j < m; ++j) {
          r += (double)w[j];
          cdf[j + 1] = (float)r;
        }
      }
    }
  }
  __syncthreads();
  if (lane < n_new) {
    const float u = linspace_at((float)(0.5 / (double)n_new), (float)(1.0 - 0.5 / (double)n_new), n_new, lane);
    int lo = 0, hi = n;
    while (lo < hi) {
      const int mid = (lo + hi) >> 1;
      if (!(cdf[mid] > u)) lo = mid + 1; else hi = mid;
    }
    const int ind = lo;
    const int below = max(ind - 1, 0);
    const int above = min(n - 1, ind);
    const float c0 = cdf[below], c1 = cdf[above];
    const float b0 = z[below], b1 = z[above];
    float denom = c1 - c0;
    if (denom < 1e-5f) denom = 1.0f;
    const float t = (u - c0) / denom;
    const float v = b0 + t * (b1 - b0);
    nz[lane] = v;
    if (a.inds) a.inds[b * n_new + lane] = ind;
    if (a.new_z) a.new_z[b * n_new + lane] = v;
    if (a.new_pts) {
      float* p = a.new_pts + (b * n_new + lane) * 3;
      p[0] = o0 + d0 * v; p[1] = o1 + d1 * v; p[2] = o2 + d2 * v;
    }
  }
  __syncthreads();
  const int nt = n + n_new;
  for (int j = lane; j < nt; j += 64) {
    a.z_out[b * nt + j] = __builtin_nanf("");
    if (a.sort_index) a.sort_index[b * nt + j] = 0;
  }
  __syncthreads();
  for (int j = lane; j < n; j += 64) {
    const float zz = z[j];
    int cnt = 0;
    for (int k = 0; k < n_new; ++k) cnt += lt_total(nz[k], zz) ? 1 : 0;
    const int pos = j + cnt;
    a.z_out[b * nt + pos] = zz;
    if (a.sort_index) a.sort_index[b * nt + pos] = j;
  }
  if (lane < n_new) {
    const float v = nz[lane];
    int lo = 0, hi = n;
    while (lo < hi) {
      const int mid = (lo + hi) >> 1;
      if (!lt_total(v, z[mid])) lo = mid + 1; else hi = mid;
    }
    int cnt = lo;
    for (int k = 0; k < n_new; ++k) cnt += (lt_total(nz[k], v) || (!lt_total(v, nz[k]) && k < lane)) ? 1 : 0;
    a.z_out[b * nt + cnt] = v;
    if (a.sort_index) a.sort_index[b * nt + cnt] = n + lane;
  }
}

__global__ void gather_sdf_kernel(const float* __restrict__ sdf_old, const float* __restrict__ sdf_new,
                                  const int32_t* __restrict__ index, int64_t B, int n, int n_new,
                                  float* __restrict__ out) {
  int64_t i = (int64_t)blockIdx.x * blockDim.x + threadIdx.x;
  const int nt = n + n_new;
  if (i >= B * nt) return;
  const int64_t b = i / nt;
  const int idx = min(max(index[i], 0), nt - 1);
  out[i] = idx < n ? sdf_old[b * n + idx] : sdf_new[b * n_new + (idx - n)];
}

int launch_z_init(const float* rays_o, const float* rays_d, const float* near, const float* far,
                  const float* t_rand, int64_t B, int n, float* z, float* pts, hipStream_t s) {
  const int64_t tot = B * n;
  hipLaunchKernelGGL(z_init_kernel, dim3((unsigned)((tot + 255) / 256)), dim3(256), 0, s, rays_o, rays_d, near, far,
                     t_rand, B, n, z, pts);
  RNB_CHECK_LAUNCH();
  return RNB_OK;
}

int launch_up_sample_step(const float* rays_o, const float* rays_d, const float* z_in, const float* sdf_old,
                          const float* sdf_new, const int32_t* gather_index, int n_old_for_gather, int64_t B,
                          int n, int n_new, float inv_s, float* new_z, int32_t* inds, float* z_out,
                          int32_t* sort_index, float* new_pts, float* sdf_sorted_out, hipStream_t s) {
  if (n < 2 || n_new < 1 || n_new > kMaxNew || n + n_new > kMaxZ)
    RNB_FAIL(RNB_E_INVALID, "up_sample: unsupported sizes n=%d n_new=%d (n_new <= %d, n+n_new <= %d)", n, n_new,
             kMaxNew, kMaxZ);
  UpArgs a{rays_o, rays_d, z_in, sdf_old, sdf_new, gather_index, gather_index ? n_old_for_gather : n, n, n_new,
           inv_s, new_z, inds, z_out, sort_index, new_pts, sdf_sorted_out};
  hipLaunchKernelGGL(up_sample_kernel, dim3((unsigned)B), dim3(64), 0, s, a);
  RNB_CHECK_LAUNCH();
  return RNB_OK;
}

int launch_gather_sdf(const float* sdf_old, const float* sdf_new, const int32_t* index, int64_t B, int n, int n_new,
                      float* out, hipStream_t s) {
  const int64_t tot = B * (n + n_new);
  hipLaunchKernelGGL(gather_sdf_kernel, dim3((unsigned)((tot + 255) / 256)), dim3(256), 0, s, sdf_old, sdf_new, index,
                     B, n, n_new, out);
  RNB_CHECK_LAUNCH();
  return RNB_OK;
}

}
```

rnb-neus-fork_amd/csrc/sweep_mv.hip:

```cpp
#include <type_traits>

#include "fused_common.hip.h"

namespace rnb {

constexpr int MV_MW = 4;
constexpr int MV_PT = 32 * MV_MW;
constexpr int MV_PIECE = 1024;
constexpr int MV_SLOT = 8 * 3 * MV_PIECE;
constexpr int MV_NSLOT = 4;
constexpr int MV_ACCP = 36;
constexpr int MV_ACC_BYTES = 32 * MV_ACCP * 4;
constexpr int MV_PLS = 3 * 1024 + 32;
constexpr int MV_PLN = 3;
constexpr int MV_PAIR_BYTES = MV_ACC_BYTES + MV_PLN * MV_PLS;
constexpr int MV_EP = 68;
constexpr int MV_SYNC = 4;
constexpr int MV_MAXM = RNB_MAX_LIN + 1;
constexpr int MV_MAXB = 8;

__host__ __device__ constexpr int mv_kfeat(int j, int r, int h) { return 32 * j + 4 * h + (r & 3) + 8 * (r >> 2); }

struct MvStream {
  int nmat;
// ... 480 lines not shown
    const bool hidden = pi < g.net.nh;
    MvEpi e = epi(hidden ? pi : 0);
#pragma unroll
    for (int b = 0; b < 8; ++b) mv_v_drain(v, pr, nblk, vacc[b], lane);
    if (hidden && pi + 1 < nprod) {
      mv_v_act<SAVE, 2>(v, e, 0, 0, vacc[0], sk, act, sacc);
      mv_v_act<SAVE, 2>(v, e, 0, 2, vacc[0], sk, act, sacc);
      if (v.c >= 4) {
#pragma unroll
        for (int i = 0; i < 4; ++i) mv_put_planes(v, (nslot0 + 1) % MV_PLN, i, act[i]);
      }
      asm volatile("s_waitcnt lgkmcnt(0)" ::: "memory");
      mv_signal(pr.sync + 2, pi + 1, lane);
    }
    gs = nslot0;
    if (pi + 1 >= nprod) {
      if (hidden) {
#pragma unroll
        for (int j = 0; j < 8; ++j) {
          mv_v_act<SAVE, 2>(v, e, j, 0, vacc[j], sk, act, sacc);
          mv_v_act<SAVE, 2>(v, e, j, 2, vacc[j], sk, act, sacc);
        }
      } else {
        const float* bf = g.packed + g.net.bf_off + 4 * v.c;
#pragma unroll
        for (int j = 0; j < 8; ++j) {
          const vf4 bv = *reinterpret_cast<const vf4*>(bf + 32 * j);
          if (32 * j + 4 * v.c < g.net.F) {
#pragma unroll
            for (int i = 0; i < 4; ++i)
              __builtin_nontemporal_store(vacc[j][i] + bv, reinterpret_cast<vf4*>(g.cin + v.row[i] * g.net.Cinp + 32 * j + 4 * v.c));
          }
        }
      }
      break;
    }
    vbar();
    mv_v_act<SAVE, 2>(v, e, 1, 0, vacc[1], sk, act, sacc);
    mv_v_act<SAVE, 2>(v, e, 1, 2, vacc[1], sk, act, sacc);
    task_planes(1, nslot0);
#pragma unroll
    for (int j = 2; j < 8; ++j) {
      vbar();
      pin(vacc[j][0]); pin(vacc[j][1]);
      mv_v_act<SAVE, 2>(v, e, j, 0, vacc[j], sk, act, sacc);
      pin_act(0); pin_act(1);
      vbar();
      pin(vacc[j][2]); pin(vacc[j][3]);
      mv_v_act<SAVE, 2>(v, e, j, 2, vacc[j], sk, act, sacc);
      task_planes(j, nslot0);
    }
    vbar();
    vbar();
    vbar();
  }
#pragma unroll
  for (int i = 0; i < 4; ++i) {
    float s = sacc[i];
    s += __shfl_xor(s, 1, 64);
    s += __shfl_xor(s, 2, 64);
    s += __shfl_xor(s, 4, 64);
    if (v.c == 0) {
      float val = (s + g.packed[g.net.bsdf_off]) / g.net.scale;
      if (*(LDSP(volatile int))(pr.sync + 3) != 0) val = __builtin_nanf("");
      if (!g.grid.on) g.sdf[v.row[i]] = val;
      else {
        const int64_t o = grid_out_index(g.grid, v.row[i], g.M);
        if (o >= 0) g.sdf[o] = val * g.grid.out_scale;
      }
    }
  }
}

bool sweep_mv_supported(const Layout& L) {
  if (!is_x3(L) || !fused_supported(L)) return false;
  if (L.Ep != 64 || L.hid[0].Kp != 64) return false;
  if (L.nh < 2 || L.nh > MV_MAXB) return false;
  for (int l = 0; l < L.nh; ++l)
    if (L.hid[l].N < 192) return false;
  if (L.F > 0 && (L.feat.Np != FH || L.feat.Kp != FH || (L.F & 3))) return false;
  return true;
}

int sweep_mv_forward(const Layout& L, const float* packed, const float* pts, int64_t M, PointBufs& pb, bool save,
                     bool need_feat, hipStream_t s, const GridGen* grid) {
  if (save) RNB_FAIL(RNB_E_INVALID, "M/V forward: forward-only sweeps only");
  MvFwdArgs ga;
  memset(&ga, 0, sizeof(ga));
  FusedFwdArgs& g = ga.f;
  g.net = sdf_net_args(L);
  if (grid) g.grid = *grid;
  g.pts = pts;
  g.M = M;
  g.packed = packed;
  g.w3 = reinterpret_cast<const x3raw*>(packed + L.total);
  ga.st.nmat = L.nh + (need_feat ? 1 : 0);
  for (int i = 0; i < ga.st.nmat; ++i) {
    const Lin& ln = i < L.nh ? L.hid[i] : L.feat;
    ga.st.nks[i] = ln.Kp / 16;
    ga.st.boff[i] = (unsigned)(6 * ln.w_off);
  }
  for (int l = 0; l < L.nh; ++l) {
    g.a[l] = pb.a[l];
    g.D[l] = pb.D[l];
  }
  g.with_feat = need_feat ? 1 : 0;
  g.cin = pb.cin;
  g.sdf = pb.sdf;
  g.x4 = pb.x;
  g.e = pb.e;
  ProfScope prof(sdf_sweep_flops(L, M, 0, true, need_feat), s, save ? "F_sweep(save)" : "F_sweep(forward_only)");
  const dim3 blocks((unsigned)(pb.Mp / MV_PT)), threads(128 * MV_MW);
  if (save) hipLaunchKernelGGL((sweep_mv_forward_kernel<true>), blocks, threads, 0, s, ga);
  else hipLaunchKernelGGL((sweep_mv_forward_kernel<false>), blocks, threads, 0, s, ga);
  RNB_CHECK_LAUNCH();
  return RNB_OK;
}

}
```

rnb-neus-fork_amd/csrc/train.hip:

```cpp
#include "rnb_internal.h"

namespace rnb {

__device__ inline double block_sum(double v, double* red) {
#pragma unroll
  for (int o = 32; o > 0; o >>= 1) v += __shfl_xor(v, o, 64);
  const int wave = threadIdx.x >> 6, lane = threadIdx.x & 63;
  __syncthreads();
  if (lane == 0) red[wave] = v;
  __syncthreads();
  double s = 0.0;
  for (int w = 0; w < (int)(blockDim.x >> 6); ++w) s += red[w];
  return s;
}

__global__ __launch_bounds__(1024) void rnb_loss_kernel(const float* __restrict__ color, const float* __restrict__ rgb,
                                                        const float* __restrict__ mask, const float* __restrict__ wsum,
                                                        const float* __restrict__ gerr, int L, int64_t B, int Cd,
                                                        float igr_w, float mask_w,
                                                        const float* __restrict__ batch_global, float eik_share, float* __restrict__ loss,
                                                        float* __restrict__ parts,
                                                        float* __restrict__ dcolor, float* __restrict__ dwsum,
                                                        float* __restrict__ dgerr) {
  __shared__ double red[16];
  const int tid = threadIdx.x, nt = blockDim.x;
  const float B_global = batch_global ? batch_global[1] : (float)B;
  double msum = 0.0, bce = 0.0;
  for (int64_t b = tid; b < B; b += nt) {
    const float m = mask_w > 0.f ? (mask[b] > 0.5f ? 1.f : 0.f) : 1.f;
    msum += m;
    const float w = wsum[b];
    const float x = clamp_nan(w, 1e-3f, 1.f - 1e-3f);
    const float lx = max_nan(logf(x), -100.f), l1x = max_nan(logf(1.f - x), -100.f);
    bce -= (double)(m * lx + (1.f - m) * l1x);
    const bool pass = w >= 1e-3f && w <= 1.f - 1e-3f;
    const float d = (x - m) / fmaxf((1.f - x) * x, 1e-12f);
    dwsum[b] = pass ? mask_w * d / B_global : 0.f;
  }
  msum = block_sum(msum, red);
  bce = block_sum(bce, red);
  const float mask_sum = (batch_global ? batch_global[0] : (float)msum) + 1e-5f;
  const float inv = 1.f / (mask_sum * (float)L);
  double l1 = 0.0;
  const int64_t n = (int64_t)L * B * Cd;
  for (int64_t i = tid; i < n; i += nt) {
    const int64_t b = (i / Cd) % B;
    const float m = mask_w > 0.f ? (mask[b] > 0.5f ? 1.f : 0.f) : 1.f;
    const float e = (color[i] - rgb[i]) * m;
    l1 += (double)fabsf(e);
    const float sg = e > 0.f ? 1.f : (e < 0.f ? -1.f : 0.f);
    dcolor[i] = sg * m * inv;
  }
  l1 = block_sum(l1, red);
  if (tid == 0) {
    const float color_loss = (float)l1 * inv;
    const float mask_loss = (float)(bce / (double)B_global);
    const float eik = gerr[0] * eik_share;
    loss[0] = color_loss + eik * igr_w + mask_loss * mask_w;
    parts[0] = color_loss;
    parts[1] = eik;
    parts[2] = mask_loss;
    dgerr[0] = igr_w;
  }
}

__global__ void adam_kernel(float* __restrict__ p, const float* __restrict__ g, float* __restrict__ m,
                            float* __restrict__ v, int64_t n, float lr, float b1, float b2, float eps, float wd,
                            float bc1, float bc2_sqrt) {
  const int64_t i = (int64_t)blockIdx.x * blockDim.x + threadIdx.x;
  if (i >= n) return;
  float grad = g[i];
  const float param = p[i];
  if (wd != 0.f) grad += wd * param;
  float ea = m[i], es = v[i];
  ea = ea + (1.f - b1) * (grad - ea);
  es = b2 * es + (1.f - b2) * grad * grad;
  const float step_size = lr / bc1;
  const float denom = sqrtf(es) / bc2_sqrt + eps;
  p[i] = param - step_size * ea / denom;
  m[i] = ea;
  v[i] = es;
}

}

#define RNB_API extern "C" __attribute__((visibility("default")))

RNB_API int rnb_loss_rnb(const float* color_fine, const float* true_rgb, const float* mask, const float* weight_sum,
                         const float* gradient_error, int32_t n_lights, int64_t B, int32_t color_depth,
                         float igr_weight, float mask_weight, float* loss, float* parts,
                         float* d_color_fine, float* d_weight_sum, float* d_gradient_error, rnb_stream_t stream) {
  using namespace rnb;
  if (!color_fine || !true_rgb || !mask || !weight_sum || !gradient_error || !loss || !parts || !d_color_fine ||
      !d_weight_sum || !d_gradient_error)
    RNB_FAIL(RNB_E_NULL, "rnb_loss_rnb: NULL pointer");
  if (n_lights < 1 || B < 1 || color_depth < 1) RNB_FAIL(RNB_E_INVALID, "rnb_loss_rnb: empty shape");
  hipLaunchKernelGGL(rnb_loss_kernel, dim3(1), dim3(1024), 0, (hipStream_t)stream, color_fine, true_rgb, mask,
                     weight_sum, gradient_error, n_lights, B, color_depth, igr_weight, mask_weight,
                     (const float*)nullptr, 1.f, loss, parts, d_color_fine, d_weight_sum, d_gradient_error);
  RNB_CHECK_LAUNCH();
  return RNB_OK;
}

RNB_API int rnb_loss_rnb_shard(const float* color_fine, const float* true_rgb, const float* mask,
                               const float* weight_sum, const float* gradient_error, int32_t n_lights, int64_t B,
                               int32_t color_depth, float igr_weight, float mask_weight, const float* batch_global,
                               float eik_share, float* loss, float* parts, float* d_color_fine,
                               float* d_weight_sum, float* d_gradient_error, rnb_stream_t stream) {
  using namespace rnb;
  if (!color_fine || !true_rgb || !mask || !weight_sum || !gradient_error || !loss || !parts || !d_color_fine ||
      !d_weight_sum || !d_gradient_error || !batch_global)
    RNB_FAIL(RNB_E_NULL, "rnb_loss_rnb_shard: NULL pointer");
  if (n_lights < 1 || B < 1 || color_depth < 1) RNB_FAIL(RNB_E_INVALID, "rnb_loss_rnb_shard: bad shape");
  hipLaunchKernelGGL(rnb_loss_kernel, dim3(1), dim3(1024), 0, (hipStream_t)stream, color_fine, true_rgb, mask,
                     weight_sum, gradient_error, n_lights, B, color_depth, igr_weight, mask_weight, batch_global,
                     eik_share, loss, parts, d_color_fine, d_weight_sum, d_gradient_error);
  RNB_CHECK_LAUNCH();
  return RNB_OK;
}

RNB_API int rnb_adam_step(float* param, const float* grad, float* exp_avg, float* exp_avg_sq, int64_t n, double lr,
                          double beta1, double beta2, double eps, double weight_decay, int64_t step,
                          rnb_stream_t stream) {
  using namespace rnb;
  if (!param || !grad || !exp_avg || !exp_avg_sq) RNB_FAIL(RNB_E_NULL, "rnb_adam_step: NULL pointer");
  if (n < 0 || step < 1) RNB_FAIL(RNB_E_INVALID, "rnb_adam_step: n %lld, step %lld", (long long)n, (long long)step);
  if (n == 0) return RNB_OK;
  const double bc1 = 1.0 - pow(beta1, (double)step);
  const double bc2 = 1.0 - pow(beta2, (double)step);
  hipLaunchKernelGGL(adam_kernel, dim3((unsigned)((n + 255) / 256)), dim3(256), 0, (hipStream_t)stream, param, grad,
                     exp_avg, exp_avg_sq, n, (float)lr, (float)beta1, (float)beta2, (float)eps, (float)weight_decay,
                     (float)bc1, (float)sqrt(bc2));
  RNB_CHECK_LAUNCH();
  return RNB_OK;
}
```

rnb-neus-fork_amd/csrc/weightnorm.hip:

```cpp
#include "rnb_internal.h"

namespace rnb {

struct WnEntry {
  const float* g;
  const float* v;
  const float* b;
  float* dg;
  float* dv;
  float* db;
  int src_row0;
  int N;
  int Nrows;
  int K, Kp;
  int row_begin;
  int cmap_f;
  int cmap_2pev;
  long long w_off, b_off;
  long long wT_off;
  float scale;
  int skip;
};
__device__ inline double wn_scale(const WnEntry& en) { return en.skip ? 0.70710678118654752440 : (double)en.scale; }
constexpr int kMaxEntries = 2 * RNB_MAX_LIN + 2;
struct WnTable {
  int n;
  int total_rows;
  WnEntry e[kMaxEntries];
};

__device__ inline int cmap(const WnEntry& en, int i) {
  if (en.cmap_f <= 0) return i;
  return i < en.cmap_2pev ? en.cmap_f + i : i - en.cmap_2pev;
}

__device__ inline float block_sum(float v, float* red) {
#pragma unroll
  for (int o = 32; o > 0; o >>= 1) v += __shfl_xor(v, o, 64);
  const int w = threadIdx.x >> 6;
  __syncthreads();
  if ((threadIdx.x & 63) == 0) red[w] = v;
  __syncthreads();
  float t = 0.f;
  for (int i = 0; i < (int)(blockDim.x >> 6); ++i) t += red[i];
  return t;
}

__device__ inline double block_sum_f64(double v, double* red) {
#pragma unroll
  for (int o = 32; o > 0; o >>= 1) v += __shfl_xor(v, o, 64);
  const int w = threadIdx.x >> 6;
  __syncthreads();
  if ((threadIdx.x & 63) == 0) red[w] = v;
  __syncthreads();
  double t = 0.0;
  for (int i = 0; i < (int)(blockDim.x >> 6); ++i) t += red[i];
  return t;
}

__global__ __launch_bounds__(256) void wn_fwd_kernel(WnTable tab, float* __restrict__ packed, unsigned* __restrict__ wmax_zero) {
  __shared__ double red[4];
  if (wmax_zero != nullptr && blockIdx.x == 0 && threadIdx.x < kH2TabSlots) wmax_zero[threadIdx.x] = 0u;
  int ei = 0;
  while (ei + 1 < tab.n && (int)blockIdx.x >= tab.e[ei + 1].row_begin) ++ei;
  const WnEntry& en = tab.e[ei];
  const int r = blockIdx.x - en.row_begin;
  float* wrow = packed + en.w_off + (long long)r * en.Kp;
  float* wT = en.wT_off >= 0 ? packed + en.wT_off + r : nullptr;
  if (r >= en.N) {
    for (int c = threadIdx.x; c < en.Kp; c += blockDim.x) {
      wrow[c] = 0.f;
      if (wT) wT[(long long)c * en.Nrows] = 0.f;
    }
    if (threadIdx.x == 0) packed[en.b_off + r] = 0.f;
    return;
  }
  const int src = en.src_row0 + r;
  const float* vrow = en.v + (long long)src * en.K;
  const double scale = wn_scale(en);
  double mult = scale;
  if (en.g != nullptr) {
    double ss = 0.0;
    for (int i = threadIdx.x; i < en.K; i += blockDim.x) ss = fma((double)vrow[i], (double)vrow[i], ss);
    ss = block_sum_f64(ss, red);
    mult = scale * ((double)en.g[src] / sqrt(ss));
  }
  for (int i = threadIdx.x; i < en.K; i += blockDim.x) {
    const int c = cmap(en, i);
    const float w = (float)((double)vrow[i] * mult);
    wrow[c] = w;
    if (wT) wT[(long long)c * en.Nrows] = w;
  }
  for (int c = en.K + threadIdx.x; c < en.Kp; c += blockDim.x) {
    wrow[c] = 0.f;
    if (wT) wT[(long long)c * en.Nrows] = 0.f;
  }
  if (threadIdx.x == 0) packed[en.b_off + r] = en.b[src];
}

__global__ __launch_bounds__(256) void wn_bwd_kernel(WnTable tab, const float* __restrict__ pgrad) {
  __shared__ double red[4];
  int ei = 0;
  while (ei + 1 < tab.n && (int)blockIdx.x >= tab.e[ei + 1].row_begin) ++ei;
  const WnEntry& en = tab.e[ei];
  const int r = blockIdx.x - en.row_begin;
  if (r >= en.N) return;
  const int src = en.src_row0 + r;
  const float* vrow = en.v + (long long)src * en.K;
  const float* dwrow = pgrad + en.w_off + (long long)r * en.Kp;
  float* dvrow = en.dv + (long long)src * en.K;
  const double scale = wn_scale(en);
  if (en.g == nullptr) {
    for (int i = threadIdx.x; i < en.K; i += blockDim.x) dvrow[i] = (float)(scale * (double)dwrow[cmap(en, i)]);
  } else {
    double ss = 0.0, t = 0.0;
    for (int i = threadIdx.x; i < en.K; i += blockDim.x) {
      const double vv = (double)vrow[i];
      ss = fma(vv, vv, ss);
      t = fma((double)dwrow[cmap(en, i)], vv, t);
    }
    ss = block_sum_f64(ss, red);
    t = block_sum_f64(t, red);
    const double inv_norm = 1.0 / sqrt(ss);
    const double coef = scale * (double)en.g[src] * inv_norm;
    const double proj = t * inv_norm * inv_norm;
    for (int i = threadIdx.x; i < en.K; i += blockDim.x)
      dvrow[i] = (float)(coef * ((double)dwrow[cmap(en, i)] - (double)vrow[i] * proj));
    if (threadIdx.x == 0) en.dg[src] = (float)(scale * t * inv_norm);
  }
  if (threadIdx.x == 0) en.db[src] = pgrad[en.b_off + r];
}

static void add_entry(WnTable& t, const rnb_mlp_params* p, const rnb_mlp_grads* g, int lin, bool wn, int src_row0,
                      int N, int Nrows, int K, int Kp, long long w_off, long long b_off, float scale, int cmap_f,
                      int cmap_2pev, long long wT_off = -1, int skip = 0) {
  WnEntry& e = t.e[t.n];
  e.g = wn ? p->g[lin] : nullptr;
  e.v = p->v[lin];
  e.b = p->b[lin];
  e.dg = (g && wn) ? g->g[lin] : nullptr;
  e.dv = g ? g->v[lin] : nullptr;
  e.db = g ? g->b[lin] : nullptr;
  e.src_row0 = src_row0;
  e.N = N;
  e.Nrows = Nrows;
  e.K = K;
  e.Kp = Kp;
  e.row_begin = t.total_rows;
  e.cmap_f = cmap_f;
  e.cmap_2pev = cmap_2pev;
  e.w_off = w_off;
  e.wT_off = wT_off;
  e.b_off = b_off;
  e.scale = scale;
  e.skip = skip;
  t.total_rows += Nrows;
  t.n++;
}

static int build_table(const rnb_model_desc* d, const Layout& L, const rnb_mlp_params* sdf,
                       const rnb_mlp_params* color, const rnb_mlp_grads* gs, const rnb_mlp_grads* gc, WnTable& t) {
  t.n = 0;
  t.total_rows = 0;
  if (!sdf && !color) RNB_FAIL(RNB_E_NULL, "both parameter sets are NULL");
  if (sdf) {
    if (sdf->n_lin != L.nh + 1) RNB_FAIL(RNB_E_INVALID, "sdf params: n_lin %d != %d", sdf->n_lin, L.nh + 1);
    const bool wn = d->sdf_weight_norm != 0;
    for (int l = 0; l <= L.nh; ++l)
      if (!sdf->v[l] || !sdf->b[l] || (wn && !sdf->g[l])) RNB_FAIL(RNB_E_NULL, "sdf lin%d has a NULL leaf", l);
    for (int l = 0; l < L.nh; ++l) {
      const Lin& ln = L.hid[l];
      add_entry(t, sdf, gs, l, wn, 0, ln.N, ln.Np, ln.K, ln.Kp, ln.w_off, ln.b_off, ln.scale, 0, 0, ln.wT_off, l == L.skip ? 1 : 0);
    }
    add_entry(t, sdf, gs, L.nh, wn, 0, 1, 1, L.H, L.Hp, L.wsdf_off, L.bsdf_off, 1.f, 0, 0);
    if (L.F > 0)
      add_entry(t, sdf, gs, L.nh, wn, 1, L.F, L.feat.Np, L.H, L.feat.Kp, L.feat.w_off, L.feat.b_off, 1.f, 0, 0,
                L.feat.wT_off);
  }
  if (color) {
    if (L.F <= 0) RNB_FAIL(RNB_E_INVALID, "albedo network needs a feature head");
    if (color->n_lin != L.nc + 1) RNB_FAIL(RNB_E_INVALID, "color params: n_lin %d != %d", color->n_lin, L.nc + 1);
    const bool wc = d->col_weight_norm != 0;
    for (int l = 0; l <= L.nc; ++l)
      if (!color->v[l] || !color->b[l] || (wc && !color->g[l])) RNB_FAIL(RNB_E_NULL, "color lin%d has a NULL leaf", l);
    for (int l = 0; l < L.nc; ++l) {
      const Lin& ln = L.col[l];
      add_entry(t, color, gc, l, wc, 0, ln.N, ln.Np, ln.K, ln.Kp, ln.w_off, ln.b_off, 1.f, l == 0 ? L.F : 0,
                l == 0 ? 2 * L.pev : 0, ln.wT_off);
    }
    add_entry(t, color, gc, L.nc, wc, 0, L.colo.N, L.colo.Np, L.colo.K, L.colo.Kp, L.colo.w_off, L.colo.b_off, 1.f, 0, 0);
  }
  return RNB_OK;
}

int weightnorm_fwd(const rnb_model_desc* d, const Layout& L, const rnb_mlp_params* sdf, const rnb_mlp_params* color,
                   float* packed, hipStream_t s) {
  WnTable t;
  RNB_TRY(build_table(d, L, sdf, color, nullptr, nullptr, t));
  H2Tab* h2 = h2_tab(L, packed);
  hipLaunchKernelGGL(wn_fwd_kernel, dim3(t.total_rows), dim3(256), 0, s, t, packed, h2 ? h2->wmax : (unsigned*)nullptr);
  RNB_CHECK_LAUNCH();
  return RNB_OK;
}

int weightnorm_bwd(const rnb_model_desc* d, const Layout& L, const rnb_mlp_params* sdf, const rnb_mlp_params* color,
                   const float* pgrad, const rnb_mlp_grads* gs, const rnb_mlp_grads* gc, hipStream_t s) {
  if (sdf && !gs) RNB_FAIL(RNB_E_NULL, "sdf grads are NULL");
  if (color && !gc) RNB_FAIL(RNB_E_NULL, "color grads are NULL");
  WnTable t;
  RNB_TRY(build_table(d, L, sdf, color, gs, gc, t));
  for (int i = 0; i < t.n; ++i)
    if (!t.e[i].dv || !t.e[i].db || (t.e[i].g && !t.e[i].dg)) RNB_FAIL(RNB_E_NULL, "a gradient leaf is NULL");
  hipLaunchKernelGGL(wn_bwd_kernel, dim3(t.total_rows), dim3(256), 0, s, t, pgrad);
  RNB_CHECK_LAUNCH();
  return RNB_OK;
}

}
```

rnb-neus-fork_amd/native.py:

```python
from __future__ import annotations

import ctypes as C
import os

_HERE = os.path.dirname(os.path.abspath(__file__))
LIB_PATH = os.path.join(_HERE, "librnbneus_hip.so")
ABI_VERSION = 5
MAX_LIN = 16

MODE_CORE = 0
MODE_MVPS = 1
FLAG_RELU_SHADING = 2
FLAG_NO_ALBEDO = 4
FLAG_LIGHT_PER_RAY = 8
FLAG_FORWARD_ONLY = 16
FLAG_INPUT_GRADS = 32
MAX_RENDER_LIGHTS = 8

POINTS_FEATURE = 1
POINTS_NORMAL = 2
POINTS_COLOR = 4

VARIANT_BF16 = 1
VARIANT_DETERMINISTIC = 2
# ... 13 lines not shown

class ModelDesc(C.Structure):
    _fields_ = [
        ("sdf_d_in", C.c_int32), ("sdf_d_out", C.c_int32), ("sdf_d_hidden", C.c_int32),
        ("sdf_n_layers", C.c_int32), ("sdf_skip_in", C.c_int32), ("sdf_multires", C.c_int32),
        ("sdf_scale", C.c_float), ("sdf_weight_norm", C.c_int32),
        ("col_d_feature", C.c_int32), ("col_d_in", C.c_int32), ("col_d_out", C.c_int32),
        ("col_d_hidden", C.c_int32), ("col_n_layers", C.c_int32), ("col_multires_view", C.c_int32),
        ("col_squeeze_out", C.c_int32), ("col_weight_norm", C.c_int32),
        ("n_samples", C.c_int32), ("n_importance", C.c_int32), ("up_sample_steps", C.c_int32),
        ("variant", C.c_int32),
    ]


class MlpParams(C.Structure):
    _fields_ = [("n_lin", C.c_int32), ("pad_", C.c_int32),
                ("g", C.c_void_p * MAX_LIN), ("v", C.c_void_p * MAX_LIN), ("b", C.c_void_p * MAX_LIN)]


MlpGrads = MlpParams


class RenderArgs(C.Structure):
    _fields_ = [
        ("B", C.c_int64), ("S", C.c_int32), ("n_lights", C.c_int32), ("flags", C.c_int32),
        ("cos_anneal_ratio", C.c_float),
        ("rays_o", C.c_void_p), ("rays_d", C.c_void_p), ("z_vals", C.c_void_p), ("lights_dir", C.c_void_p),
        ("background_rgb", C.c_void_p), ("variance", C.c_void_p),
        ("color_fine", C.c_void_p), ("weights", C.c_void_p), ("cdf_fine", C.c_void_p),
        ("gradients", C.c_void_p), ("inside_sphere", C.c_void_p), ("weight_sum", C.c_void_p),
        ("weight_max", C.c_void_p), ("s_val", C.c_void_p), ("gradient_error", C.c_void_p),
        ("sdf", C.c_void_p), ("sampled_albedo", C.c_void_p),
        ("gerr_partial", C.c_void_p), ("gerr_den_global", C.c_void_p),
    ]


class RenderMapsOut(C.Structure):
    _fields_ = [("color", C.c_void_p), ("normal", C.c_void_p), ("albedo", C.c_void_p), ("depth", C.c_void_p),
                ("weight_sum", C.c_void_p), ("weight_max", C.c_void_p)]


class GridDesc(C.Structure):
    _fields_ = [("bound_min", C.c_float * 3), ("bound_max", C.c_float * 3), ("resolution", C.c_int32),
                ("x_begin", C.c_int32), ("x_end", C.c_int32), ("out_scale", C.c_float)]


class SparseGridDesc(C.Structure):
    _fields_ = [("brick", C.c_int32), ("threshold", C.c_float), ("margin", C.c_float)]


SPARSE_BRICKS = (4, 8, 16, 32)


def brick_geometry(res: int, brick: int) -> dict:
    res, brick = int(res), int(brick)
    if res < 2:
        raise ValueError(f"a grid of resolution {res} has no cells")
    if brick not in SPARSE_BRICKS:
        raise ValueError(f"brick must be one of {SPARSE_BRICKS}, not {brick}")
    nb = (res - 1 + brick - 1) // brick
    n1 = brick + 1
    return {"nb": nb, "lattice": [min(k * brick, res - 1) for k in range(nb + 1)], "samples": n1,
            "rows": (n1 ** 3 + 63) // 64 * 64, "bricks_total": nb ** 3}


class RenderGrads(C.Structure):
    _fields_ = [("color_fine", C.c_void_p), ("weights", C.c_void_p), ("cdf_fine", C.c_void_p),
                ("gradients", C.c_void_p), ("weight_sum", C.c_void_p), ("weight_max", C.c_void_p),
                ("s_val", C.c_void_p), ("gradient_error", C.c_void_p)]


class RenderInputGrads(C.Structure):
    _fields_ = [("rays_o", C.c_void_p), ("rays_d", C.c_void_p), ("lights_dir", C.c_void_p),
                ("background_rgb", C.c_void_p), ("z_vals", C.c_void_p)]


_P = C.POINTER
_SIGNATURES = {
    "rnb_abi_version": (C.c_int, []),
    "rnb_last_error_string": (C.c_char_p, []),
    "rnb_build_id": (C.c_char_p, []),
    "rnb_packed_floats": (C.c_int, [_P(ModelDesc), _P(C.c_int64)]),
    "rnb_weightnorm_fwd": (C.c_int, [_P(ModelDesc), _P(MlpParams), _P(MlpParams), C.c_void_p, C.c_void_p]),
    "rnb_weightnorm_bwd": (C.c_int, [_P(ModelDesc), _P(MlpParams), _P(MlpParams), C.c_void_p, _P(MlpGrads),
                                     _P(MlpGrads), C.c_void_p]),
    "rnb_points_workspace_bytes": (C.c_int, [_P(ModelDesc), C.c_int64, _P(C.c_int64)]),
    "rnb_sdf_forward": (C.c_int, [_P(ModelDesc), C.c_void_p, C.c_void_p, C.c_int64, C.c_void_p, C.c_void_p,
                                  C.c_void_p, C.c_size_t, C.c_void_p]),
    "rnb_sdf_gradient": (C.c_int, [_P(ModelDesc), C.c_void_p, C.c_void_p, C.c_int64, C.c_void_p, C.c_void_p,
                                   C.c_void_p, C.c_size_t, C.c_void_p]),
    "rnb_color_forward": (C.c_int, [_P(ModelDesc), C.c_void_p, C.c_void_p, C.c_void_p, C.c_void_p, C.c_int64,
                                    C.c_void_p, C.c_void_p, C.c_size_t, C.c_void_p]),
    "rnb_points_grad_workspace_bytes": (C.c_int, [_P(ModelDesc), C.c_int64, C.c_int32, _P(C.c_int64)]),
    "rnb_sdf_forward_save": (C.c_int, [_P(ModelDesc), C.c_void_p, C.c_void_p, C.c_int64, C.c_int32, C.c_void_p,
                                       C.c_void_p, C.c_void_p, C.c_void_p, C.c_size_t, C.c_void_p]),
    "rnb_sdf_backward": (C.c_int, [_P(ModelDesc), C.c_void_p, C.c_int64, C.c_int32, C.c_void_p, C.c_void_p,
                                   C.c_void_p, C.c_void_p, C.c_void_p, C.c_void_p, C.c_size_t, C.c_void_p]),
    "rnb_color_forward_save": (C.c_int, [_P(ModelDesc), C.c_void_p, C.c_void_p, C.c_void_p, C.c_void_p, C.c_int64,
                                         C.c_void_p, C.c_void_p, C.c_size_t, C.c_void_p]),
    "rnb_color_backward": (C.c_int, [_P(ModelDesc), C.c_void_p, C.c_int64, C.c_void_p, C.c_void_p, C.c_void_p,
                                     C.c_void_p, C.c_void_p, C.c_void_p, C.c_size_t, C.c_void_p]),
    "rnb_sdf_grid_workspace_bytes": (C.c_int, [_P(ModelDesc), _P(GridDesc), _P(C.c_int64)]),
    "rnb_sdf_grid": (C.c_int, [_P(ModelDesc), C.c_void_p, _P(GridDesc), C.c_void_p, C.c_void_p, C.c_size_t,
                               C.c_void_p]),
    "rnb_sdf_grid_sparse_workspace_bytes": (C.c_int, [_P(ModelDesc), _P(GridDesc), _P(SparseGridDesc), _P(C.c_int64)]),
    "rnb_sdf_grid_sparse_seed": (C.c_int, [_P(ModelDesc), C.c_void_p, _P(GridDesc), _P(SparseGridDesc), C.c_void_p,
                                           C.c_size_t, C.c_void_p, C.c_void_p]),
    "rnb_sdf_grid_sparse_round": (C.c_int, [_P(ModelDesc), C.c_void_p, _P(GridDesc), _P(SparseGridDesc), C.c_void_p,
                                            C.c_void_p, C.c_size_t, C.c_int64, C.c_int64, C.c_void_p, C.c_void_p]),
    "rnb_sdf_grid_sparse_finish": (C.c_int, [_P(ModelDesc), _P(GridDesc), _P(SparseGridDesc), C.c_void_p, C.c_void_p,
                                             C.c_size_t, C.c_void_p, C.c_void_p]),
    "rnb_marching_cubes_workspace_bytes": (C.c_int, [C.c_int32, C.c_int32, C.c_int32, _P(C.c_int64)]),
    "rnb_marching_cubes_count": (C.c_int, [C.c_void_p, C.c_int32, C.c_int32, C.c_int32, C.c_float, C.c_void_p,
                                           C.c_size_t, C.c_void_p, C.c_void_p]),
    "rnb_marching_cubes_emit": (C.c_int, [C.c_void_p, C.c_int32, C.c_int32, C.c_int32, C.c_float, C.c_void_p,
                                          C.c_size_t, C.c_int64, C.c_int64, C.c_void_p, C.c_void_p, C.c_void_p]),
    "rnb_up_sample_step": (C.c_int, [C.c_void_p, C.c_void_p, C.c_void_p, C.c_void_p, C.c_int64, C.c_int32,
                                     C.c_int32, C.c_float, C.c_void_p, C.c_void_p, C.c_void_p, C.c_void_p,
                                     C.c_void_p]),
    "rnb_gather_sdf": (C.c_int, [C.c_void_p, C.c_void_p, C.c_void_p, C.c_int64, C.c_int32, C.c_int32,
                                 C.c_void_p, C.c_void_p]),
    "rnb_sample_workspace_bytes": (C.c_int, [_P(ModelDesc), C.c_int64, _P(C.c_int64)]),
    "rnb_sample_rays": (C.c_int, [_P(ModelDesc), C.c_void_p, C.c_void_p, C.c_void_p, C.c_void_p, C.c_void_p,
                                  C.c_void_p, C.c_int64, C.c_void_p, C.c_void_p, C.c_size_t, C.c_void_p]),
    "rnb_render_workspace_bytes": (C.c_int, [_P(ModelDesc), C.c_int64, C.c_int32, C.c_int32, _P(C.c_int64)]),
    "rnb_render_fwd": (C.c_int, [_P(ModelDesc), C.c_void_p, _P(RenderArgs), C.c_void_p, C.c_size_t, C.c_void_p]),
    "rnb_render_maps": (C.c_int, [_P(ModelDesc), C.c_void_p, _P(RenderArgs), _P(RenderMapsOut), C.c_void_p, C.c_size_t,
                                  C.c_void_p]),
    "rnb_render_bwd": (C.c_int, [_P(ModelDesc), C.c_void_p, _P(RenderArgs), _P(RenderGrads), C.c_void_p,
                                 C.c_void_p, C.c_void_p, C.c_size_t, C.c_void_p]),
    "rnb_render_bwd_inputs": (C.c_int, [_P(ModelDesc), C.c_void_p, _P(RenderArgs), _P(RenderGrads),
                                        _P(RenderInputGrads), C.c_void_p, C.c_void_p, C.c_void_p, C.c_size_t,
                                        C.c_void_p]),
    "rnb_render_range": (C.c_int, [_P(ModelDesc), C.c_void_p, C.c_void_p, C.c_size_t, C.c_int64, C.c_int32, C.c_int32,
                                   C.c_void_p, C.c_void_p]),
    "rnb_algorithmic_flops": (C.c_int, [_P(ModelDesc), C.c_int64, C.c_int32, _P(C.c_double), _P(C.c_double)]),
    "rnb_algorithmic_bytes": (C.c_int, [_P(ModelDesc), C.c_int64, C.c_int32, _P(C.c_double)]),
    "rnb_gen_rays_at_view": (C.c_int, [C.c_void_p, C.c_void_p, C.c_void_p, C.c_void_p, C.c_void_p, C.c_int32,
                                       C.c_void_p, C.c_void_p, C.c_void_p, C.c_int64, C.c_int32, C.c_int32,
                                       C.c_int32, C.c_void_p, C.c_void_p, C.c_void_p, C.c_void_p, C.c_void_p,
                                       C.c_void_p, C.c_void_p]),
    "rnb_gen_rays_grid": (C.c_int, [C.c_void_p, C.c_void_p, C.c_void_p, C.c_void_p, C.c_int32, C.c_int32, C.c_int64,
                                    C.c_int64, C.c_void_p, C.c_void_p, C.c_void_p, C.c_int32, C.c_void_p, C.c_int32,
                                    C.c_int32, C.c_int32, C.c_int32, C.c_void_p, C.c_void_p, C.c_void_p, C.c_void_p,
                                    C.c_void_p, C.c_void_p, C.c_void_p]),
    "rnb_loss_rnb": (C.c_int, [C.c_void_p, C.c_void_p, C.c_void_p, C.c_void_p, C.c_void_p, C.c_int32, C.c_int64,
                               C.c_int32, C.c_float, C.c_float, C.c_void_p, C.c_void_p, C.c_void_p, C.c_void_p,
                               C.c_void_p, C.c_void_p]),
    "rnb_loss_rnb_shard": (C.c_int, [C.c_void_p, C.c_void_p, C.c_void_p, C.c_void_p, C.c_void_p, C.c_int32, C.c_int64,
                                     C.c_int32, C.c_float, C.c_float, C.c_void_p, C.c_float, C.c_void_p,
                                     C.c_void_p, C.c_void_p, C.c_void_p, C.c_void_p, C.c_void_p]),
    "rnb_adam_step": (C.c_int, [C.c_void_p, C.c_void_p, C.c_void_p, C.c_void_p, C.c_int64, C.c_double, C.c_double,
                                C.c_double, C.c_double, C.c_double, C.c_int64, C.c_void_p]),
    "rnb_profile_enable": (C.c_int, [C.c_int]),
    "rnb_profile_collect": (C.c_int, [_P(C.c_double), _P(C.c_int64), _P(C.c_double)]),
    "rnb_profile_report": (C.c_int64, [C.c_char_p, C.c_int64]),
}

EXPORTED_SYMBOLS = tuple(_SIGNATURES.keys())

_lib = None


class NativeError(RuntimeError):
    pass

# ... 85 lines not shown
```

Before: 204,900 rays/s.

## Pack only consumed x3 weight mirrors and tighten several reduction kernels

The x3 weight-packing step now works out which weight mirrors (hidden, feature, color, transposed or not) the active kernels actually read, and writes only those. It still scans all non-transposed blocks for the maxima that x2h needs. Alongside this, several reductions change: weightnorm runs 64-thread blocks with shuffle reductions, the split-K dW reduction uses vectorized non-temporal loads, the composite forward uses fused wave shuffles and the backward precomputes its suffix-sum terms, and the loss kernel prefetches its inputs and merges two block sums. Unroll hints are also raised in the sampling and sdf-head loops. The main risk is that a later consumer reads a mirror that was skipped, which would give stale weights.

After: 206,600 rays/s (median of 6 runs). About the same (+0.9%).

```diff
diff --git a/include/rnbneus.h b/include/rnbneus.h
--- a/include/rnbneus.h
+++ b/include/rnbneus.h
@@ -88,6 +88,12 @@
 int rnb_weightnorm_bwd(const rnb_model_desc* desc, const rnb_mlp_params* sdf, const rnb_mlp_params* color,
                        const float* packed_grad, const rnb_mlp_grads* sdf_grads,
                        const rnb_mlp_grads* color_grads, rnb_stream_t stream);
+enum {
+  RNB_X3S_HID_W = 1, RNB_X3S_HID_WT = 2,
+  RNB_X3S_FEAT_W = 4, RNB_X3S_FEAT_WT = 8,
+  RNB_X3S_COL_W = 16, RNB_X3S_COL_WT = 32
+};
+int rnb_x3_mirror_sets(const rnb_model_desc* desc, int32_t* packed_set, int32_t* read_set);
 
 int rnb_points_workspace_bytes(const rnb_model_desc* desc, int64_t n_points, int64_t* bytes);
 int rnb_sdf_forward(const rnb_model_desc* desc, const float* packed, const float* pts, int64_t n,
diff --git a/rnb-neus-fork_amd/csrc/api.hip b/rnb-neus-fork_amd/csrc/api.hip
--- a/rnb-neus-fork_amd/csrc/api.hip
+++ b/rnb-neus-fork_amd/csrc/api.hip
@@ -37,6 +37,16 @@
   RNB_TRY(weightnorm_fwd(desc, L, sdf, color, packed, (hipStream_t)stream));
   if (is_bf16(L)) RNB_TRY(bf16_pack_weights(L, packed, (hipStream_t)stream));
   if (is_x3(L)) RNB_TRY(x3_pack_weights(L, packed, (hipStream_t)stream));
+  return RNB_OK;
+}
+
+RNB_API int rnb_x3_mirror_sets(const rnb_model_desc* desc, int32_t* packed_set, int32_t* read_set) {
+  RNB_REQUIRE(packed_set, "packed_set");
+  RNB_REQUIRE(read_set, "read_set");
+  Layout L;
+  RNB_TRY(make_layout(desc, &L));
+  *packed_set = (int32_t)x3_mirror_packed(L);
+  *read_set = (int32_t)(is_x3(L) ? x3_mirror_reads(L) : 0u);
   return RNB_OK;
 }
 
diff --git a/rnb-neus-fork_amd/csrc/backward.hip b/rnb-neus-fork_amd/csrc/backward.hip
--- a/rnb-neus-fork_amd/csrc/backward.hip
+++ b/rnb-neus-fork_amd/csrc/backward.hip
@@ -76,7 +76,7 @@
   const int64_t r0 = (int64_t)blockIdx.x * rows_per_blk;
   const int64_t r1 = min(M, r0 + rows_per_blk);
   double s[4] = {0.0, 0.0, 0.0, 0.0}, sb = 0.0;
-#pragma unroll 4
+#pragma unroll 8
   for (int64_t row = r0 + ph; row < r1; row += 64) {
     const float t = sbar[row] * inv_scale;
     if (cg == 0) sb += (double)t;
diff --git a/rnb-neus-fork_amd/csrc/composite.hip b/rnb-neus-fork_amd/csrc/composite.hip
--- a/rnb-neus-fork_amd/csrc/composite.hip
+++ b/rnb-neus-fork_amd/csrc/composite.hip
@@ -141,22 +141,39 @@
       }
     }
   }
-  wsum = wave_sum(wsum);
-  wmax = wave_max(wmax);
-  gnum = wave_sum(gnum);
-  gden = wave_sum(gden);
+#pragma unroll
+  for (int o = 32; o > 0; o >>= 1) {
+    const float t0 = __shfl_xor(wsum, o, 64), t1 = __shfl_xor(wmax, o, 64), t2 = __shfl_xor(gnum, o, 64),
+                t3 = __shfl_xor(gden, o, 64);
+    wsum += t0;
+    wmax = max_nan(wmax, t1);
+    gnum += t2;
+    gden += t3;
+  }
   const int nl = mvps ? a.L : 1;
-  for (int l = 0; l < nl; ++l)
-    for (int c = 0; c < a.C; ++c) {
-      float v = wave_sum(col[l][c]);
-      if (lane == 0) {
-        if (mvps) a.color_fine[((int64_t)l * a.B + b) * a.C + c] = v;
-        else if (c < 3) {
-          if (a.bg) v += a.bg[c] * (1.0f - wsum);
-          a.color_fine[b * 3 + c] = v;
-        }
-      }
-    }
+#pragma unroll
+  for (int l = 0; l < kMaxL; ++l) {
+    if (l >= nl) break;
+    float v[4];
+#pragma unroll
+    for (int c = 0; c < 4; ++c) v[c] = col[l][c];
+#pragma unroll
+    for (int o = 32; o > 0; o >>= 1) {
+      float t[4];
+#pragma unroll
+      for (int c = 0; c < 4; ++c) t[c] = __shfl_xor(v[c], o, 64);
+#pragma unroll
+      for (int c = 0; c < 4; ++c) v[c] += t[c];
+    }
+    if (lane == 0) {
+#pragma unroll
+      for (int c = 0; c < 4; ++c) {
+        if (c >= a.C) break;
+        if (mvps) a.color_fine[((int64_t)l * a.B + b) * a.C + c] = v[c];
+        else if (c < 3) a.color_fine[b * 3 + c] = a.bg ? v[c] + a.bg[c] * (1.0f - wsum) : v[c];
+      }
+    }
+  }
   if (lane == 0) {
     a.weight_sum[b] = wsum;
     a.weight_max[b] = wmax;
@@ -300,6 +317,7 @@
 template <bool IG>
 __device__ __forceinline__ void composite_bwd_body(const CompBwdArgs& g) {
   __shared__ float sAlpha[kMaxS], sT[kMaxS], sWbar[kMaxS], sSuf[kMaxS];
+  __shared__ double sTerm[kMaxS];
   if (g.amax_to_zero != nullptr && blockIdx.x == 0) {
     static_assert(AMAX_SLOTS <= 64, "one wave zeroes the slots");
     if ((int)threadIdx.x < AMAX_SLOTS) g.amax_to_zero[threadIdx.x] = 0u;
@@ -417,11 +435,24 @@
     if (lane == 0 && cand < S) sWbar[cand] += g_wmax;
   }
   __syncthreads();
+  for (int j = lane; j < S; j += 64) sTerm[j] = (double)sWbar[j] * (double)(sAlpha[j] * sT[j]);
+  __syncthreads();
   if (lane == 0) {
     double run = 0.0;
-    for (int j = S - 1; j >= 0; --j) {
+    int j = S - 1;
+    for (; j >= 7; j -= 8) {
+      double t[8];
+#pragma unroll
+      for (int u = 0; u < 8; ++u) t[u] = sTerm[j - u];
+#pragma unroll
+      for (int u = 0; u < 8; ++u) {
+        sSuf[j - u] = (float)run;
+        run += t[u];
+      }
+    }
+    for (; j >= 0; --j) {
       sSuf[j] = (float)run;
-      run += (double)sWbar[j] * (double)(sAlpha[j] * sT[j]);
+      run += sTerm[j];
     }
   }
   __syncthreads();
diff --git a/rnb-neus-fork_amd/csrc/dw.hip.h b/rnb-neus-fork_amd/csrc/dw.hip.h
--- a/rnb-neus-fork_amd/csrc/dw.hip.h
+++ b/rnb-neus-fork_amd/csrc/dw.hip.h
@@ -286,21 +286,75 @@
     }
     return;
   }
-  for (size_t idx = (size_t)blockIdx.x * 256 + threadIdx.x; idx < n; idx += (size_t)gridDim.x * 256) {
-    double s[4] = {0.0, 0.0, 0.0, 0.0};
-    int sp = 0;
-    for (; sp + 4 <= J.splits; sp += 4) {
-#pragma unroll
-      for (int u = 0; u < 4; ++u) s[u] += (double)J.part[(size_t)(sp + u) * n + idx];
-    }
-    for (int u = 0; sp < J.splits; ++sp, ++u) s[u] += (double)J.part[(size_t)sp * n + idx];
-    const size_t dst = dense ? idx : (idx / (size_t)J.K) * (size_t)J.lddw + idx % (size_t)J.K;
-    J.dW[dst] = (float)((s[0] + s[1]) + (s[2] + s[3]));
+  if ((n & 3) == 0 && (J.K & 3) == 0 && (J.lddw & 3) == 0 && (((size_t)J.part | (size_t)J.dW) & 15) == 0) {
+    const size_t n4 = n >> 2;
+    for (size_t i4 = (size_t)blockIdx.x * 256 + threadIdx.x; i4 < n4; i4 += (size_t)gridDim.x * 256) {
+      const vf4* src = reinterpret_cast<const vf4*>(J.part) + i4;
+      double s[4][4];
+#pragma unroll
+      for (int u = 0; u < 4; ++u)
+#pragma unroll
+        for (int e = 0; e < 4; ++e) s[u][e] = 0.0;
+      int sp = 0;
+      for (; sp + 16 <= J.splits; sp += 16) {
+        vf4 v[16];
+#pragma unroll
+        for (int q = 0; q < 16; ++q) v[q] = __builtin_nontemporal_load(src + (size_t)(sp + q) * n4);
+#pragma unroll
+        for (int q = 0; q < 16; ++q)
+#pragma unroll
+          for (int e = 0; e < 4; ++e) s[q & 3][e] += (double)v[q][e];
+      }
+      for (; sp + 4 <= J.splits; sp += 4) {
+        vf4 v[4];
+#pragma unroll
+        for (int u = 0; u < 4; ++u) v[u] = __builtin_nontemporal_load(src + (size_t)(sp + u) * n4);
+#pragma unroll
+        for (int u = 0; u < 4; ++u)
+#pragma unroll
+          for (int e = 0; e < 4; ++e) s[u][e] += (double)v[u][e];
+      }
+      for (int u = 0; sp < J.splits; ++sp, ++u) {
+        const vf4 v = __builtin_nontemporal_load(src + (size_t)sp * n4);
+#pragma unroll
+        for (int e = 0; e < 4; ++e) {
+          if (u == 0) s[0][e] += (double)v[e];
+          else if (u == 1) s[1][e] += (double)v[e];
+          else s[2][e] += (double)v[e];
+        }
+      }
+      vf4 out;
+#pragma unroll
+      for (int e = 0; e < 4; ++e) out[e] = (float)((s[0][e] + s[1][e]) + (s[2][e] + s[3][e]));
+      const size_t idx = i4 << 2;
+      const size_t dst = dense ? idx : (idx / (size_t)J.K) * (size_t)J.lddw + idx % (size_t)J.K;
+      *reinterpret_cast<vf4*>(J.dW + dst) = out;
+    }
+  } else {
+    for (size_t idx = (size_t)blockIdx.x * 256 + threadIdx.x; idx < n; idx += (size_t)gridDim.x * 256) {
+      double s[4] = {0.0, 0.0, 0.0, 0.0};
+      int sp = 0;
+      for (; sp + 4 <= J.splits; sp += 4) {
+#pragma unroll
+        for (int u = 0; u < 4; ++u) s[u] += (double)J.part[(size_t)(sp + u) * n + idx];
+      }
+      for (int u = 0; sp < J.splits; ++sp, ++u) s[u] += (double)J.part[(size_t)sp * n + idx];
+      const size_t dst = dense ? idx : (idx / (size_t)J.K) * (size_t)J.lddw + idx % (size_t)J.K;
+      J.dW[dst] = (float)((s[0] + s[1]) + (s[2] + s[3]));
+    }
   }
   if (J.db != nullptr && J.partb != nullptr) {
     for (int r = blockIdx.x * 256 + threadIdx.x; r < J.N; r += gridDim.x * 256) {
       double s = 0.0;
-      for (int sp = 0; sp < J.splits; ++sp) s += (double)J.partb[(size_t)sp * J.N + r];
+      int sp = 0;
+      for (; sp + 8 <= J.splits; sp += 8) {
+        float v[8];
+#pragma unroll
+        for (int q = 0; q < 8; ++q) v[q] = J.partb[(size_t)(sp + q) * J.N + r];
+#pragma unroll
+        for (int q = 0; q < 8; ++q) s += (double)v[q];
+      }
+      for (; sp < J.splits; ++sp) s += (double)J.partb[(size_t)sp * J.N + r];
       J.db[r] = (float)s;
     }
   }
diff --git a/rnb-neus-fork_amd/csrc/fused.hip b/rnb-neus-fork_amd/csrc/fused.hip
--- a/rnb-neus-fork_amd/csrc/fused.hip
+++ b/rnb-neus-fork_amd/csrc/fused.hip
@@ -250,7 +250,7 @@
 }
 
 constexpr int kMaxX3 = 4 * RNB_MAX_LIN + 2;
-struct X3Entry { long long off; int N, K, unit_begin, tperm, id, tr; };
+struct X3Entry { long long off; int N, K, unit_begin, tperm, id, tr; unsigned cls; int store; };
 struct X3Table { int n, total_units; X3Entry e[kMaxX3]; };
 __global__ __launch_bounds__(256) void x3_pack_kernel(const float* __restrict__ src, X3Table t, x3raw* __restrict__ dst,
                                                       H2Tab* __restrict__ tab) {
@@ -269,12 +269,14 @@
     const int c = lane & 31, h = lane >> 5;
     const float* sp = src + en.off + (size_t)(nt * 32 + c) * en.K + ks * 16 + h * (en.tperm ? 4 : 8);
     const vf4 x0 = *reinterpret_cast<const vf4*>(sp), x1 = *reinterpret_cast<const vf4*>(sp + (en.tperm ? 8 : 4));
-    vu4x hi, mid, lo;
-    x3_split8(x0, x1, hi, mid, lo);
-    x3raw* dp = dst + 3 * en.off + ((size_t)frag * 3 * 64 + lane) * 8;
-    *reinterpret_cast<vu4x*>(dp) = hi;
-    *reinterpret_cast<vu4x*>(dp + 512) = mid;
-    *reinterpret_cast<vu4x*>(dp + 1024) = lo;
+    if (en.store) {
+      vu4x hi, mid, lo;
+      x3_split8(x0, x1, hi, mid, lo);
+      x3raw* dp = dst + 3 * en.off + ((size_t)frag * 3 * 64 + lane) * 8;
+      *reinterpret_cast<vu4x*>(dp) = hi;
+      *reinterpret_cast<vu4x*>(dp + 512) = mid;
+      *reinterpret_cast<vu4x*>(dp + 1024) = lo;
+    }
     m = fmaxf(fmaxf(fmaxf(fabsf(x0.x), fabsf(x0.y)), fmaxf(fabsf(x0.z), fabsf(x0.w))),
               fmaxf(fmaxf(fabsf(x1.x), fabsf(x1.y)), fmaxf(fabsf(x1.z), fabsf(x1.w))));
   }
@@ -320,35 +322,58 @@
   *reinterpret_cast<vu4x*>(dp) = hi;
   *reinterpret_cast<vu4x*>(dp + 512) = lo;
 }
-int x3_pack_weights(const Layout& L, float* packed, hipStream_t s) {
-  x3raw* dst = reinterpret_cast<x3raw*>(packed + L.total);
+unsigned fused_forward_x3_reads(const Layout& L) {
+  if (!is_x3(L)) return 0;
+  return (is_x2h(L) ? 0u : (X3S_HID_W | (L.F > 0 ? X3S_FEAT_W : 0u))) | sweep_mv_x3_reads(L);
+}
+unsigned x3_mirror_reads(const Layout& L) {
+  return fused_forward_x3_reads(L) | fused_bwd_x3_reads(L) | layers_x3_reads(L);
+}
+static X3Table x3_table(const Layout& L, unsigned stored, bool maxima) {
   X3Table t;
   t.n = 0;
   t.total_units = 0;
-  auto add = [&](long long off, int N, int K, int tperm, int id, int tr) {
+  auto add = [&](long long off, int N, int K, int tperm, int id, int tr, unsigned cls) {
     if (off < 0 || N <= 0 || K <= 0) return;
+    const bool st = (stored & cls) != 0;
+    if (!st && !(maxima && !tr)) return;
     X3Entry& e = t.e[t.n++];
     e.off = off; e.N = N; e.K = K; e.unit_begin = t.total_units; e.tperm = tperm; e.id = id; e.tr = tr;
+    e.cls = cls; e.store = st ? 1 : 0;
     t.total_units += N * K / 8;
   };
   for (int l = 0; l < L.nh; ++l) {
-    add(L.hid[l].w_off, L.hid[l].Np, L.hid[l].Kp, 1, l, 0);
-    add(L.hid[l].wT_off, L.hid[l].Kp, L.hid[l].Np, 1, l, 1);
+    add(L.hid[l].w_off, L.hid[l].Np, L.hid[l].Kp, 1, l, 0, X3S_HID_W);
+    add(L.hid[l].wT_off, L.hid[l].Kp, L.hid[l].Np, 1, l, 1, X3S_HID_WT);
   }
   if (L.F > 0) {
-    add(L.feat.w_off, L.feat.Np, L.feat.Kp, 1, L.nh, 0);
-    add(L.feat.wT_off, L.feat.Kp, L.feat.Np, 1, L.nh, 1);
+    add(L.feat.w_off, L.feat.Np, L.feat.Kp, 1, L.nh, 0, X3S_FEAT_W);
+    add(L.feat.wT_off, L.feat.Kp, L.feat.Np, 1, L.nh, 1, X3S_FEAT_WT);
   }
   for (int l = 0; l < L.nc; ++l) {
-    add(L.col[l].w_off, L.col[l].Np, L.col[l].Kp, 0, L.nh + 1 + l, 0);
-    add(L.col[l].wT_off, L.col[l].Kp, L.col[l].Np, 0, L.nh + 1 + l, 1);
-  }
+    add(L.col[l].w_off, L.col[l].Np, L.col[l].Kp, 0, L.nh + 1 + l, 0, X3S_COL_W);
+    add(L.col[l].wT_off, L.col[l].Kp, L.col[l].Np, 0, L.nh + 1 + l, 1, X3S_COL_WT);
+  }
+  return t;
+}
+unsigned x3_mirror_packed(const Layout& L) {
+  if (!is_x3(L)) return 0;
+  const X3Table t = x3_table(L, x3_mirror_reads(L), is_x2h(L));
+  unsigned set = 0;
+  for (int q = 0; q < t.n; ++q)
+    if (t.e[q].store) set |= t.e[q].cls;
+  return set;
+}
+int x3_pack_weights(const Layout& L, float* packed, hipStream_t s) {
+  x3raw* dst = reinterpret_cast<x3raw*>(packed + L.total);
+  const X3Table t = x3_table(L, x3_mirror_reads(L), is_x2h(L));
   H2Tab* tab = is_x2h(L) ? h2_tab(L, packed) : nullptr;
-  hipLaunchKernelGGL(x3_pack_kernel, dim3((unsigned)((t.total_units + 255) / 256)), dim3(256), 0, s, packed, t, dst, tab);
+  if (t.total_units > 0) hipLaunchKernelGGL(x3_pack_kernel, dim3((unsigned)((t.total_units + 255) / 256)), dim3(256), 0, s, packed, t, dst, tab);
   RNB_CHECK_LAUNCH();
   if (is_x2h(L)) {
-    for (int q = 0; q < t.n; ++q) t.e[q].tperm = 1;
-    hipLaunchKernelGGL(x2h_pack_kernel, dim3((unsigned)((t.total_units + 255) / 256)), dim3(256), 0, s, packed, t,
+    X3Table t2 = x3_table(L, X3S_ALL, false);
+    for (int q = 0; q < t2.n; ++q) t2.e[q].tperm = 1;
+    hipLaunchKernelGGL(x2h_pack_kernel, dim3((unsigned)((t2.total_units + 255) / 256)), dim3(256), 0, s, packed, t2,
                        x2h_mirror(L, packed), tab);
     RNB_CHECK_LAUNCH();
   }
diff --git a/rnb-neus-fork_amd/csrc/fused_bwd.hip b/rnb-neus-fork_amd/csrc/fused_bwd.hip
--- a/rnb-neus-fork_amd/csrc/fused_bwd.hip
+++ b/rnb-neus-fork_amd/csrc/fused_bwd.hip
@@ -538,6 +538,16 @@
   });
 }
 
+unsigned fused_bwd_x3_reads(const Layout& L) {
+  if (!is_x3(L)) return 0;
+  unsigned set = X3S_HID_W;
+  if (!is_x2h(L)) set |= X3S_HID_WT;
+  const int kt = L.knob(RNB_VARIANT_BWD_TI_SHIFT);
+  const int ti = kt == 1 || kt == 2 ? kt : 2;
+  if (!(is_x2h(L) && ti == 2)) set |= X3S_HID_WT | (L.F > 0 ? X3S_FEAT_WT : 0u);
+  return set;
+}
+
 int fused_reverse(const Layout& L, const float* packed, PointBufs& pb, hipStream_t s, bool store_ge) {
   FusedBwdArgs g;
   fill_args(L, packed, pb, g);
diff --git a/rnb-neus-fork_amd/csrc/layers.hip b/rnb-neus-fork_amd/csrc/layers.hip
--- a/rnb-neus-fork_amd/csrc/layers.hip
+++ b/rnb-neus-fork_amd/csrc/layers.hip
@@ -467,6 +467,11 @@
 static inline const x3raw* x3_mirror(const Layout& L, const float* packed, int64_t off) {
   if (!is_x3(L) || off < 0) return nullptr;
   return reinterpret_cast<const x3raw*>(packed + L.total) + 3 * off;
+}
+
+unsigned layers_x3_reads(const Layout& L) {
+  if (!is_x3(L) || L.F <= 0) return 0;
+  return X3S_COL_W | (L.route.color == COLOR_LAYERS ? X3S_COL_WT : 0u);
 }
 
 int launch_pe_points(const Layout& L, const float* pts, int64_t M, PointBufs& pb, hipStream_t s) {
diff --git a/rnb-neus-fork_amd/csrc/rnb_internal.h b/rnb-neus-fork_amd/csrc/rnb_internal.h
--- a/rnb-neus-fork_amd/csrc/rnb_internal.h
+++ b/rnb-neus-fork_amd/csrc/rnb_internal.h
@@ -382,6 +382,18 @@
   return L.h2tab_off >= 0 ? reinterpret_cast<H2Tab*>(packed + L.h2tab_off) : nullptr;
 }
 int x3_pack_weights(const Layout& L, float* packed, hipStream_t s);
+enum : unsigned {
+  X3S_HID_W = RNB_X3S_HID_W, X3S_HID_WT = RNB_X3S_HID_WT,
+  X3S_FEAT_W = RNB_X3S_FEAT_W, X3S_FEAT_WT = RNB_X3S_FEAT_WT,
+  X3S_COL_W = RNB_X3S_COL_W, X3S_COL_WT = RNB_X3S_COL_WT,
+  X3S_ALL = 63
+};
+unsigned fused_forward_x3_reads(const Layout& L);
+unsigned sweep_mv_x3_reads(const Layout& L);
+unsigned fused_bwd_x3_reads(const Layout& L);
+unsigned layers_x3_reads(const Layout& L);
+unsigned x3_mirror_reads(const Layout& L);
+unsigned x3_mirror_packed(const Layout& L);
 
 bool color_h2_supported(const Layout& L);
 int color_h2_forward(const Layout& L, const float* packed, PointBufs& pb, const float* pts, const float* nrm, hipStream_t s);
diff --git a/rnb-neus-fork_amd/csrc/sampling.hip b/rnb-neus-fork_amd/csrc/sampling.hip
--- a/rnb-neus-fork_amd/csrc/sampling.hip
+++ b/rnb-neus-fork_amd/csrc/sampling.hip
@@ -197,6 +197,7 @@
   for (int j = lane; j < n; j += 64) {
     const float zz = z[j];
     int cnt = 0;
+#pragma unroll 8
     for (int k = 0; k < n_new; ++k) cnt += lt_total(nz[k], zz) ? 1 : 0;
     const int pos = j + cnt;
     a.z_out[b * nt + pos] = zz;
@@ -210,6 +211,7 @@
       if (!lt_total(v, z[mid])) lo = mid + 1; else hi = mid;
     }
     int cnt = lo;
+#pragma unroll 8
     for (int k = 0; k < n_new; ++k) cnt += (lt_total(nz[k], v) || (!lt_total(v, nz[k]) && k < lane)) ? 1 : 0;
     a.z_out[b * nt + cnt] = v;
     if (a.sort_index) a.sort_index[b * nt + cnt] = n + lane;
diff --git a/rnb-neus-fork_amd/csrc/sweep_mv.hip b/rnb-neus-fork_amd/csrc/sweep_mv.hip
--- a/rnb-neus-fork_amd/csrc/sweep_mv.hip
+++ b/rnb-neus-fork_amd/csrc/sweep_mv.hip
@@ -586,6 +586,12 @@
   return true;
 }
 
+unsigned sweep_mv_x3_reads(const Layout& L) {
+  if (!sweep_mv_supported(L) || (L.variant & RNB_VARIANT_LDS_TILE)) return 0;
+  if (!(L.variant & RNB_VARIANT_REG_TILE) && !kRegTileDefault) return 0;
+  return X3S_HID_W | (L.F > 0 ? X3S_FEAT_W : 0u);
+}
+
 int sweep_mv_forward(const Layout& L, const float* packed, const float* pts, int64_t M, PointBufs& pb, bool save,
                      bool need_feat, hipStream_t s, const GridGen* grid) {
   if (save) RNB_FAIL(RNB_E_INVALID, "M/V forward: forward-only sweeps only");
diff --git a/rnb-neus-fork_amd/csrc/train.hip b/rnb-neus-fork_amd/csrc/train.hip
--- a/rnb-neus-fork_amd/csrc/train.hip
+++ b/rnb-neus-fork_amd/csrc/train.hip
@@ -13,6 +13,22 @@
   for (int w = 0; w < (int)(blockDim.x >> 6); ++w) s += red[w];
   return s;
 }
+__device__ inline void block_sum2(double& a, double& b, double (*red)[16]) {
+#pragma unroll
+  for (int o = 32; o > 0; o >>= 1) {
+    const double ta = __shfl_xor(a, o, 64), tb = __shfl_xor(b, o, 64);
+    a += ta;
+    b += tb;
+  }
+  const int wave = threadIdx.x >> 6, lane = threadIdx.x & 63;
+  __syncthreads();
+  if (lane == 0) { red[0][wave] = a; red[1][wave] = b; }
+  __syncthreads();
+  double sa = 0.0, sb = 0.0;
+  for (int w = 0; w < (int)(blockDim.x >> 6); ++w) { sa += red[0][w]; sb += red[1][w]; }
+  a = sa;
+  b = sb;
+}
 
 __global__ __launch_bounds__(1024) void rnb_loss_kernel(const float* __restrict__ color, const float* __restrict__ rgb,
                                                         const float* __restrict__ mask, const float* __restrict__ wsum,
@@ -22,9 +38,27 @@
                                                         float* __restrict__ parts,
                                                         float* __restrict__ dcolor, float* __restrict__ dwsum,
                                                         float* __restrict__ dgerr) {
-  __shared__ double red[16];
+  __shared__ double red[2][16];
   const int tid = threadIdx.x, nt = blockDim.x;
   const float B_global = batch_global ? batch_global[1] : (float)B;
+  constexpr int kPre = 8;
+  const int64_t n = (int64_t)L * B * Cd;
+  const bool pre = n <= (int64_t)kPre * nt;
+  float pc[kPre], pr[kPre], pm[kPre];
+  if (pre) {
+    const unsigned Bu = (unsigned)B, Cu = (unsigned)Cd;
+#pragma unroll
+    for (int k = 0; k < kPre; ++k) {
+      const unsigned i = (unsigned)tid + (unsigned)(k * nt);
+      pc[k] = pr[k] = pm[k] = 0.f;
+      if (i < (unsigned)n) {
+        pc[k] = color[i];
+        pr[k] = rgb[i];
+        pm[k] = mask[(i / Cu) % Bu];
+      }
+    }
+  }
+  const float gerr0 = gerr[0];
   double msum = 0.0, bce = 0.0;
   for (int64_t b = tid; b < B; b += nt) {
     const float m = mask_w > 0.f ? (mask[b] > 0.5f ? 1.f : 0.f) : 1.f;
@@ -37,25 +71,35 @@
     const float d = (x - m) / fmaxf((1.f - x) * x, 1e-12f);
     dwsum[b] = pass ? mask_w * d / B_global : 0.f;
   }
-  msum = block_sum(msum, red);
-  bce = block_sum(bce, red);
+  block_sum2(msum, bce, red);
   const float mask_sum = (batch_global ? batch_global[0] : (float)msum) + 1e-5f;
   const float inv = 1.f / (mask_sum * (float)L);
   double l1 = 0.0;
-  const int64_t n = (int64_t)L * B * Cd;
-  for (int64_t i = tid; i < n; i += nt) {
-    const int64_t b = (i / Cd) % B;
-    const float m = mask_w > 0.f ? (mask[b] > 0.5f ? 1.f : 0.f) : 1.f;
-    const float e = (color[i] - rgb[i]) * m;
+  auto l1_elem = [&](int64_t i, float c, float r, float mk) {
+    const float m = mask_w > 0.f ? (mk > 0.5f ? 1.f : 0.f) : 1.f;
+    const float e = (c - r) * m;
     l1 += (double)fabsf(e);
     const float sg = e > 0.f ? 1.f : (e < 0.f ? -1.f : 0.f);
     dcolor[i] = sg * m * inv;
+  };
+  auto l1_term = [&](int64_t i, int64_t b) { l1_elem(i, color[i], rgb[i], mask[b]); };
+  if (pre) {
+#pragma unroll
+    for (int k = 0; k < kPre; ++k) {
+      const unsigned i = (unsigned)tid + (unsigned)(k * nt);
+      if (i < (unsigned)n) l1_elem(i, pc[k], pr[k], pm[k]);
+    }
+  } else if (n < ((int64_t)1 << 31)) {
+    const unsigned Bu = (unsigned)B, Cu = (unsigned)Cd;
+    for (unsigned i = tid; i < (unsigned)n; i += nt) l1_term(i, (i / Cu) % Bu);
+  } else {
+    for (int64_t i = tid; i < n; i += nt) l1_term(i, (i / Cd) % B);
   }
-  l1 = block_sum(l1, red);
+  l1 = block_sum(l1, red[0]);
   if (tid == 0) {
     const float color_loss = (float)l1 * inv;
     const float mask_loss = (float)(bce / (double)B_global);
-    const float eik = gerr[0] * eik_share;
+    const float eik = gerr0 * eik_share;
     loss[0] = color_loss + eik * igr_w + mask_loss * mask_w;
     parts[0] = color_loss;
     parts[1] = eik;
diff --git a/rnb-neus-fork_amd/csrc/weightnorm.hip b/rnb-neus-fork_amd/csrc/weightnorm.hip
--- a/rnb-neus-fork_amd/csrc/weightnorm.hip
+++ b/rnb-neus-fork_amd/csrc/weightnorm.hip
@@ -58,8 +58,39 @@
   return t;
 }
 
-__global__ __launch_bounds__(256) void wn_fwd_kernel(WnTable tab, float* __restrict__ packed, unsigned* __restrict__ wmax_zero) {
-  __shared__ double red[4];
+constexpr int kWnThreads = 64;
+static_assert(kH2TabSlots <= kWnThreads, "wn_fwd_kernel's first workgroup zeroes the scale table's maxima");
+template <int NV, class F>
+__device__ inline void wn_row_sums(int K, double (&out)[NV], F&& term) {
+  double part[4][NV];
+#pragma unroll
+  for (int q = 0; q < 4; ++q) {
+#pragma unroll
+    for (int v = 0; v < NV; ++v) part[q][v] = 0.0;
+    for (int i = threadIdx.x + 64 * q; i < K; i += 256) term(i, part[q]);
+  }
+#pragma unroll
+  for (int o = 32; o > 0; o >>= 1) {
+    double t[4][NV];
+#pragma unroll
+    for (int q = 0; q < 4; ++q)
+#pragma unroll
+      for (int v = 0; v < NV; ++v) t[q][v] = __shfl_xor(part[q][v], o, 64);
+#pragma unroll
+    for (int q = 0; q < 4; ++q)
+#pragma unroll
+      for (int v = 0; v < NV; ++v) part[q][v] += t[q][v];
+  }
+#pragma unroll
+  for (int v = 0; v < NV; ++v) {
+    double tot = 0.0;
+#pragma unroll
+    for (int q = 0; q < 4; ++q) tot += part[q][v];
+    out[v] = tot;
+  }
+}
+
+__global__ __launch_bounds__(kWnThreads) void wn_fwd_kernel(WnTable tab, float* __restrict__ packed, unsigned* __restrict__ wmax_zero) {
   if (wmax_zero != nullptr && blockIdx.x == 0 && threadIdx.x < kH2TabSlots) wmax_zero[threadIdx.x] = 0u;
   int ei = 0;
   while (ei + 1 < tab.n && (int)blockIdx.x >= tab.e[ei + 1].row_begin) ++ei;
@@ -80,10 +111,9 @@
   const double scale = wn_scale(en);
   double mult = scale;
   if (en.g != nullptr) {
-    double ss = 0.0;
-    for (int i = threadIdx.x; i < en.K; i += blockDim.x) ss = fma((double)vrow[i], (double)vrow[i], ss);
-    ss = block_sum_f64(ss, red);
-    mult = scale * ((double)en.g[src] / sqrt(ss));
+    double ss[1];
+    wn_row_sums<1>(en.K, ss, [&](int i, double (&acc)[1]) { acc[0] = fma((double)vrow[i], (double)vrow[i], acc[0]); });
+    mult = scale * ((double)en.g[src] / sqrt(ss[0]));
   }
   for (int i = threadIdx.x; i < en.K; i += blockDim.x) {
     const int c = cmap(en, i);
@@ -98,8 +128,7 @@
   if (threadIdx.x == 0) packed[en.b_off + r] = en.b[src];
 }
 
-__global__ __launch_bounds__(256) void wn_bwd_kernel(WnTable tab, const float* __restrict__ pgrad) {
-  __shared__ double red[4];
+__global__ __launch_bounds__(kWnThreads) void wn_bwd_kernel(WnTable tab, const float* __restrict__ pgrad) {
   int ei = 0;
   while (ei + 1 < tab.n && (int)blockIdx.x >= tab.e[ei + 1].row_begin) ++ei;
   const WnEntry& en = tab.e[ei];
@@ -113,14 +142,13 @@
   if (en.g == nullptr) {
     for (int i = threadIdx.x; i < en.K; i += blockDim.x) dvrow[i] = (float)(scale * (double)dwrow[cmap(en, i)]);
   } else {
-    double ss = 0.0, t = 0.0;
-    for (int i = threadIdx.x; i < en.K; i += blockDim.x) {
+    double sums[2];
+    wn_row_sums<2>(en.K, sums, [&](int i, double (&acc)[2]) {
       const double vv = (double)vrow[i];
-      ss = fma(vv, vv, ss);
-      t = fma((double)dwrow[cmap(en, i)], vv, t);
-    }
-    ss = block_sum_f64(ss, red);
-    t = block_sum_f64(t, red);
+      acc[0] = fma(vv, vv, acc[0]);
+      acc[1] = fma((double)dwrow[cmap(en, i)], vv, acc[1]);
+    });
+    const double ss = sums[0], t = sums[1];
     const double inv_norm = 1.0 / sqrt(ss);
     const double coef = scale * (double)en.g[src] * inv_norm;
     const double proj = t * inv_norm * inv_norm;
@@ -198,7 +226,7 @@
   WnTable t;
   RNB_TRY(build_table(d, L, sdf, color, nullptr, nullptr, t));
   H2Tab* h2 = h2_tab(L, packed);
-  hipLaunchKernelGGL(wn_fwd_kernel, dim3(t.total_rows), dim3(256), 0, s, t, packed, h2 ? h2->wmax : (unsigned*)nullptr);
+  hipLaunchKernelGGL(wn_fwd_kernel, dim3(t.total_rows), dim3(kWnThreads), 0, s, t, packed, h2 ? h2->wmax : (unsigned*)nullptr);
   RNB_CHECK_LAUNCH();
   return RNB_OK;
 }
@@ -211,7 +239,7 @@
   RNB_TRY(build_table(d, L, sdf, color, gs, gc, t));
   for (int i = 0; i < t.n; ++i)
     if (!t.e[i].dv || !t.e[i].db || (t.e[i].g && !t.e[i].dg)) RNB_FAIL(RNB_E_NULL, "a gradient leaf is NULL");
-  hipLaunchKernelGGL(wn_bwd_kernel, dim3(t.total_rows), dim3(256), 0, s, t, pgrad);
+  hipLaunchKernelGGL(wn_bwd_kernel, dim3(t.total_rows), dim3(kWnThreads), 0, s, t, pgrad);
   RNB_CHECK_LAUNCH();
   return RNB_OK;
 }
diff --git a/rnb-neus-fork_amd/native.py b/rnb-neus-fork_amd/native.py
--- a/rnb-neus-fork_amd/native.py
+++ b/rnb-neus-fork_amd/native.py
@@ -119,6 +119,7 @@
     "rnb_build_id": (C.c_char_p, []),
     "rnb_packed_floats": (C.c_int, [_P(ModelDesc), _P(C.c_int64)]),
     "rnb_weightnorm_fwd": (C.c_int, [_P(ModelDesc), _P(MlpParams), _P(MlpParams), C.c_void_p, C.c_void_p]),
+    "rnb_x3_mirror_sets": (C.c_int, [_P(ModelDesc), _P(C.c_int32), _P(C.c_int32)]),
     "rnb_weightnorm_bwd": (C.c_int, [_P(ModelDesc), _P(MlpParams), _P(MlpParams), C.c_void_p, _P(MlpGrads),
                                      _P(MlpGrads), C.c_void_p]),
     "rnb_points_workspace_bytes": (C.c_int, [_P(ModelDesc), C.c_int64, _P(C.c_int64)]),
```
